# bobochow/adapt-image-models

Measured on AMD Instinct MI355X. Metric: clips/sec (8-frame 224^2 ViT-B/16 AIM fwd+bwd), higher is better.
Workload: dtype bf16; 1 GPU; BASELINE configs[1]: ViT-B/16 + AIM adapters, 8 frames 224^2, 64 clips/GPU, K400-shaped synthetic clips (400 random labels), fwd+bwd+AdamW; global_batch=64, frames=8, parallelism=dp1

## Files before the change

### adapt-image-models_amd/backbone.py

```python
import logging
import os
from collections import OrderedDict
from typing import Dict, List, Optional

import torch
from torch import nn

from . import ops
from .registry import BACKBONES

BF16, F32 = torch.bfloat16, torch.float32
_LOG = logging.getLogger("aim_amd")


def get_root_logger():
    return _LOG


class Adapter(nn.Module):

    def __init__(self, D_features: int, mlp_ratio: float = 0.25, skip_connect: bool = True):
        super().__init__()
        self.skip_connect = skip_connect
        hidden = int(D_features * mlp_ratio)
        self.D_fc1 = nn.Linear(D_features, hidden)
        self.D_fc2 = nn.Linear(hidden, D_features)


class LayerNorm(nn.LayerNorm):
    """Parameter container; the fp32 LayerNorm itself runs in ``aim_layernorm_fwd`` (vit_clip.py:71-77)."""


class QuickGELU(nn.Module):
    """Placeholder so ``mlp`` keeps the reference's three-entry Sequential (vit_clip.py:80-82,93-97)."""


class ResidualAttentionBlock(nn.Module):

    def __init__(self, d_model: int, n_head: int, scale: float = 1., num_frames: int = 8, drop_path: float = 0.):
        super().__init__()
        self.attn = nn.MultiheadAttention(d_model, n_head)
        self.ln_1 = LayerNorm(d_model)
        self.mlp = nn.Sequential(OrderedDict([
            ("c_fc", nn.Linear(d_model, d_model * 4)),
            ("gelu", QuickGELU()),
            ("c_proj", nn.Linear(d_model * 4, d_model))]))
        self.ln_2 = LayerNorm(d_model)
        self.n_head = n_head
        self.d_model = d_model
        self.MLP_Adapter = Adapter(d_model, skip_connect=False)
        self.S_Adapter = Adapter(d_model, skip_connect=False)
        self.scale = scale
        self.T_Adapter = Adapter(d_model, skip_connect=False)
        self.num_frames = num_frames
        self.drop_prob = float(drop_path)


class Transformer(nn.Module):
    def __init__(self, num_frames, width, layers, heads, scale=1., drop_path=0.1):
        super().__init__()
        self.width, self.layers = width, layers
        dpr = [x.item() for x in torch.linspace(0, drop_path, layers)]
        self.resblocks = nn.Sequential(*[
            ResidualAttentionBlock(width, heads, scale, num_frames, dpr[i]) for i in range(layers)])


_ADAPTERS = ("MLP_Adapter", "S_Adapter", "T_Adapter")
_ADAPTER_LEAVES = ("D_fc1.weight", "D_fc1.bias", "D_fc2.weight", "D_fc2.bias")


def _cast(w: torch.Tensor, transpose: bool = False) -> torch.Tensor:
    w2 = w.detach().reshape(w.shape[0], -1).contiguous().float()
    R, C = w2.shape
    out = torch.empty((C, R) if transpose else (R, C), dtype=BF16, device=w.device)
    ops.cast_bf16(w2, out, transpose)
    return out


class _Frozen:

    def __init__(self, blk: ResidualAttentionBlock):
        a = blk.attn
        self.Wqkv, self.WqkvT = _cast(a.in_proj_weight), _cast(a.in_proj_weight, True)
        self.Wo, self.WoT = _cast(a.out_proj.weight), _cast(a.out_proj.weight, True)
        D = blk.d_model
        r = blk.MLP_Adapter.D_fc1.weight.shape[0]
        dev = a.in_proj_weight.device
        self.D, self.r, self.H4 = D, r, 4 * D
        self.Wcat1 = torch.empty((4 * D + r, D), dtype=BF16, device=dev)
        self.Wcat2 = torch.empty((D, 4 * D + r), dtype=BF16, device=dev)
        self.WcatT2 = torch.empty((4 * D + r, D), dtype=BF16, device=dev)
        self.WcatT1 = torch.empty((D, 4 * D + r), dtype=BF16, device=dev)
        wfc, wpr = blk.mlp.c_fc.weight.detach().float().contiguous(), blk.mlp.c_proj.weight.detach().float().contiguous()
        ops.cast_bf16(wfc, self.Wcat1[:4 * D])
        ops.cast_bf16(wpr, self.Wcat2[:, :4 * D])
        ops.cast_bf16(wpr, self.WcatT2[:4 * D], transpose=True)
        ops.cast_bf16(wfc, self.WcatT1[:, :4 * D], transpose=True)
        self.bcat1 = torch.zeros(4 * D + r, dtype=F32, device=dev)
        self.bcat1[:4 * D] = blk.mlp.c_fc.bias.detach().float()
        self.small = {a: dict(W1=torch.empty((r, D), dtype=BF16, device=dev), W1T=torch.empty((D, r), dtype=BF16, device=dev),
                              W2=torch.empty((D, r), dtype=BF16, device=dev), W2T=torch.empty((r, D), dtype=BF16, device=dev))
                      for a in ("S_Adapter", "T_Adapter")}
        f = lambda p: p.detach().float().contiguous()
        self.bqkv, self.bo = f(a.in_proj_bias), f(a.out_proj.bias)
        self.bpr = f(blk.mlp.c_proj.bias)
        self.g1, self.b1 = f(blk.ln_1.weight), f(blk.ln_1.bias)
        self.g2, self.b2 = f(blk.ln_2.weight), f(blk.ln_2.bias)


    def cast_entries(self, name, w1, w2, b1=None):
        H4 = self.H4
        if name == "MLP_Adapter":
            ent = [(w1, self.Wcat1[H4:], False), (w2, self.Wcat2[:, H4:], False),
                   (w2, self.WcatT2[H4:], True), (w1, self.WcatT1[:, H4:], True)]
            if b1 is not None:
                ent.append((b1.reshape(1, -1), self.bcat1[H4:].reshape(1, -1), 2))
            return ent
        b = self.small[name]
        return [(w1, b["W1"], False), (w1, b["W1T"], True), (w2, b["W2"], False), (w2, b["W2T"], True)]

    def stage_mlp_adapter(self, w1, b1, w2, b2):
        for src, dst, tr in self.cast_entries("MLP_Adapter", w1.detach().float().contiguous(),
                                              w2.detach().float().contiguous()):
            ops.cast_bf16(src, dst, transpose=tr)
        self.stage_mlp_bias(b1, b2)

    def stage_mlp_bias(self, b1, b2, copy_b1: bool = True):
        if copy_b1:
            self.bcat1[self.H4:] = b1.detach().float()
        self.b2row = b2.detach().float().reshape(1, -1).contiguous()


class _Frozen8:

    def __init__(self, blk: ResidualAttentionBlock):
        a, ma = blk.attn, blk.MLP_Adapter
        q = ops.quantize_fp8_rows
        self.Wqkv, self.sqkv = q(a.in_proj_weight)
        self.Wo, self.so = q(a.out_proj.weight)
        self.Wcat1, self.s1 = q(torch.cat([blk.mlp.c_fc.weight.detach().float(), ma.D_fc1.weight.detach().float()], 0))
        self.Wcat2, self.s2 = q(torch.cat([blk.mlp.c_proj.weight.detach().float(), ma.D_fc2.weight.detach().float()], 1))


class _AdapterW:

    def __init__(self, w1, b1, w2, b2, bufs=None):
        if bufs is None:
            self.W1, self.W1T = _cast(w1), _cast(w1, True)
            self.W2, self.W2T = _cast(w2), _cast(w2, True)
        else:
            self.W1, self.W1T, self.W2, self.W2T = bufs["W1"], bufs["W1T"], bufs["W2"], bufs["W2T"]
        self.b1, self.b2 = b1.detach().float().contiguous(), b2.detach().float().contiguous()


def _empty(shape, dtype, dev):
    return torch.empty(shape, dtype=dtype, device=dev)


class _Arena:

    def __init__(self, dev, nbytes: int):
        self.dev, self.chunk = dev, int(nbytes)
        self.buf = torch.empty(self.chunk, dtype=torch.uint8, device=dev)
        self.off = 0
        self.main = torch.cuda.current_stream(dev) if dev.type == "cuda" else None

    def take(self, shape, dtype):
        n = 1
        for d in shape:
            n *= int(d)
        nbytes = (n * _ELEM[dtype] + 255) // 256 * 256
        if self.off + nbytes > self.buf.numel():
            with torch.cuda.stream(self.main):
                self.buf = torch.empty(max(self.chunk, nbytes), dtype=torch.uint8, device=self.dev)
            self.off = 0
        v = self.buf[self.off:self.off + nbytes].view(dtype)[:n].view(shape)
        self.off += nbytes
        return v


_ELEM = {BF16: 2, F32: 4}


_SIDE = {}
_DETACHED = {}

_JOIN_STATS = [] if os.environ.get("AIM_JOIN_STATS") else None


def join_stats():
    out = {}
    for tag, e0, e1 in _JOIN_STATS or []:
        out[tag] = out.get(tag, 0.0) + e0.elapsed_time(e1)
    if _JOIN_STATS is not None:
        _JOIN_STATS.clear()
    return out
_USE_SIDE = os.environ.get("AIM_SIDE_STREAM", "1") != "0"
_LAMBDA_ON_SIDE = os.environ.get("AIM_LAMBDA_SIDE", "1") != "0"
_LATE_JOIN = os.environ.get("AIM_LATE_JOIN", "1") != "0"
_FSUM_IN_LN = os.environ.get("AIM_FSUM_IN_LN", "1") != "0"
_CLS_EARLY = os.environ.get("AIM_CLS_EARLY", "1") != "0"
_LAMBDA_FUSED = os.environ.get("AIM_LAMBDA_FUSED", "1") != "0"
_DETACH_WGRAD = os.environ.get("AIM_DETACH_WGRAD", "1") != "0"
_DETACH_BIG = os.environ.get("AIM_DETACH_BIG", "1") != "0"
_EXPSUM_DETACHED = os.environ.get("AIM_EXPSUM_DETACHED", "0") != "0"
_DETACHED_PRIORITY = int(os.environ.get("AIM_DETACHED_PRIORITY", "0"))
_AUX_GRAD = os.environ.get("AIM_AUX_GRAD", "1") != "0"
_AUX_FRAG = os.environ.get("AIM_AUX_FRAG", "1") != "0" and os.environ.get("AIM_GEMM_TILE", "") != "128"
_DP_RESERVE = int(os.environ.get("AIM_DP_RESERVE_CUS", "0"))
_FP8_RES16 = os.environ.get("AIM_FP8_RES16", "1") != "0"
_EXPSUM_BORDER = os.environ.get("AIM_EXPSUM_BORDER", "1") != "0"
_QKV_RESERVE = int(os.environ.get("AIM_QKV_RESERVE", "32"))


class _Fork:

    def __init__(self, dev, tag: str = ""):
        self.enabled = _USE_SIDE
        self.dev = dev
        self.tag = tag
        self.started = False
        if self.enabled:
            key = (dev.type, dev.index)
            if key not in _SIDE:
                _SIDE[key] = torch.cuda.Stream(device=dev, priority=int(os.environ.get("AIM_SIDE_PRIORITY", "-1")))
            self.side_stream = _SIDE[key]
            self.main = torch.cuda.current_stream(dev)

    def sync_main_to_side(self):
        if self.enabled and self.started:
            ev = torch.cuda.Event()
            ev.record(self.side_stream)
            if _JOIN_STATS is not None:
                e0, e1 = torch.cuda.Event(enable_timing=True), torch.cuda.Event(enable_timing=True)
                e0.record(self.main)
                self.main.wait_event(ev)
                e1.record(self.main)
                _JOIN_STATS.append((self.tag + "-mid", e0, e1))
                return
            self.main.wait_event(ev)

    def sync_side_to_main(self):
        if self.enabled:
            ev = torch.cuda.Event()
            ev.record(self.main)
            self.side_stream.wait_event(ev)

    def side(self):
        fork = self

        class _Section:
            def __enter__(self_inner):
                if fork.enabled:
                    if not fork.started:
                        fork.started = True
                        fork.sync_side_to_main()
                    self_inner.ctx = torch.cuda.stream(fork.side_stream)
                    self_inner.ctx.__enter__()
                    if _JOIN_STATS is not None:
                        self_inner.t0 = torch.cuda.Event(enable_timing=True)
                        self_inner.t0.record(fork.side_stream)
                return fork

            def __exit__(self_inner, *exc):
                if fork.enabled:
                    if _JOIN_STATS is not None:
                        t1 = torch.cuda.Event(enable_timing=True)
                        t1.record(fork.side_stream)
                        _JOIN_STATS.append((fork.tag + "-span", self_inner.t0, t1))
                    self_inner.ctx.__exit__(*exc)
                return False

        return _Section()

    def __enter__(self):
        self._sec = self.side()
        return self._sec.__enter__()

    def __exit__(self, *exc):
        return self._sec.__exit__(*exc)

    def run_detached(self, calls: list, keep: list):
        if not calls:
            return
        if not (self.enabled and _DETACH_WGRAD):
            ctx = self.side() if self.enabled else None
            if ctx is not None:
                with ctx:
                    for f in calls:
                        f()
            else:
                for f in calls:
                    f()
            return
        key = (self.dev.type, self.dev.index)
        if key not in _DETACHED:
            _DETACHED[key] = torch.cuda.Stream(device=self.dev, priority=_DETACHED_PRIORITY)
        w = _DETACHED[key]
        ev = torch.cuda.Event()
        ev.record(self.side_stream)
        w.wait_event(ev)
        with torch.cuda.stream(w):
            for f in calls:
                f()
        keep.extend(calls)

    def run_beside(self, fn):
        if not self.enabled:
            fn()
            return None
        key = (self.dev.type, self.dev.index)
        if key not in _DETACHED:
            _DETACHED[key] = torch.cuda.Stream(device=self.dev, priority=_DETACHED_PRIORITY)
        w = _DETACHED[key]
        ev = torch.cuda.Event()
        ev.record(self.main)
        w.wait_event(ev)
        with torch.cuda.stream(w):
            fn()
        done = torch.cuda.Event()
        done.record(w)
        return done

    @staticmethod
    def streams(dev):
        key = (dev.type, dev.index)
        out = [torch.cuda.current_stream(dev)]
        for table in (_SIDE, _DETACHED):
            if key in table:
                out.append(table[key])
        return out

    @staticmethod
    def join_detached(dev):
        w = _DETACHED.get((dev.type, dev.index))
        if w is not None:
            ev = torch.cuda.Event()
            ev.record(w)
            main = torch.cuda.current_stream(dev)
            if _JOIN_STATS is not None:
                e0, e1 = torch.cuda.Event(enable_timing=True), torch.cuda.Event(enable_timing=True)
                e0.record(main)
                main.wait_event(ev)
                e1.record(main)
                _JOIN_STATS.append(("detached", e0, e1))
                return
            main.wait_event(ev)

    def join(self):
        if self.enabled and self.started:
            done = torch.cuda.Event()
            done.record(self.side_stream)
            if _JOIN_STATS is not None:
                e0, e1 = torch.cuda.Event(enable_timing=True), torch.cuda.Event(enable_timing=True)
                e0.record(self.main)
                self.main.wait_event(done)
                e1.record(self.main)
                _JOIN_STATS.append((self.tag, e0, e1))
                return
            self.main.wait_event(done)


def _adapter_fwd_small(x_bf, ad: _AdapterW, rows, r, D, ar: _Arena, out_f32: bool):
    pre, h = ar.take((rows, r), BF16), ar.take((rows, r), BF16)
    ops.gemm(x_bf, ad.W1, ops.EPI_ACT, h, bias=ad.b1, out2=pre, act=ops.ACT_GELU, aux_grad=_AUX_GRAD)
    out = ar.take((rows, D), F32 if out_f32 else BF16)
    ops.gemm(h, ad.W2, ops.EPI_F32 if out_f32 else ops.EPI_BF16, out, bias=ad.b2)
    return out, pre, h


def _block_forward(x, fz: _Frozen, adp: Dict[str, _AdapterW], B, T, N, H, dms1, dms2, save: bool, f8: Optional[_Frozen8] = None):
    assert f8 is None or not save
    dev = x.device
    M, D = x.shape
    BT = B * T
    r = fz.r
    fork = _Fork(dev, "fwd")
    ar = _Arena(dev, 48 * BT * D + 4 * B * H * T * T + 8 * BT * N + (1 << 16))

    def cls_chain(qkv_src, n_stride):
        ot = ar.take((BT, D), BF16)
        probs = ar.take((B, H, T, T), F32)
        ops.cls_attn_fwd(qkv_src, ot, probs, B, T, n_stride, H)
        ta = ar.take((BT, D), BF16)
        ops.gemm(ot, fz.Wo, ops.EPI_BF16, ta, bias=fz.bo)
        xt, t_pre, t_h = _adapter_fwd_small(ta, adp["T_Adapter"], BT, r, D, ar, out_f32=False)
        kv = ar.take((BT, 2 * D), BF16)
        ops.gemm(xt, fz.Wqkv[D:], ops.EPI_BF16, kv, bias=fz.bqkv[D:])
        crs = ar.take((BT, D), F32)
        ops.gemm(kv[:, D:], fz.Wo, ops.EPI_F32, crs, bias=fz.bo)
        return probs, ta, t_pre, t_h, kv, crs

    if _CLS_EARLY:
        with fork.side():
            xl_cls = ar.take((BT, D), BF16)
            if x.dtype == BF16:
                ops.layernorm_fwd_x16(x, fz.g1, fz.b1, BT, D, N * D, y_bf16=xl_cls)
            else:
                ops.layernorm_fwd(x, fz.g1, fz.b1, BT, D, N * D, y_bf16=xl_cls, mean=ar.take((BT,), F32),
                                  rstd=ar.take((BT,), F32))
            qkv_cls = ar.take((BT, 3 * D), BF16)
            ops.gemm(xl_cls, fz.Wqkv, ops.EPI_BF16, qkv_cls, bias=fz.bqkv)
            probs, ta, t_pre, t_h, kv, crs = cls_chain(qkv_cls, 1)
    qkv = _empty((M, 3 * D), BF16, dev)
    reserve = _QKV_RESERVE if (_CLS_EARLY and fork.enabled) else 0
    if f8 is not None:
        xl = _empty((M, D), ops.FP8, dev)
        mean1 = rstd1 = None
        if x.dtype == BF16:
            ops.layernorm_fwd_x16(x, fz.g1, fz.b1, M, D, D, y8=xl)
        else:
            ops.layernorm_fwd_fp8(x, fz.g1, fz.b1, M, D, D, xl)
        ops.gemm_fp8(xl, f8.Wqkv, f8.sqkv, ops.EPI_BF16, qkv, bias=fz.bqkv, reserve_cus=reserve)
    else:
        xl = _empty((M, D), BF16, dev)
        mean1, rstd1 = _empty((M,), F32, dev), _empty((M,), F32, dev)
        ops.layernorm_fwd(x, fz.g1, fz.b1, M, D, D, y_bf16=xl, mean=mean1, rstd=rstd1)
        ops.gemm(xl, fz.Wqkv, ops.EPI_BF16, qkv, bias=fz.bqkv, reserve_cus=reserve)
    del xl
    if not _CLS_EARLY:
        with fork.side():
            probs, ta, t_pre, t_h, kv, crs = cls_chain(qkv, N)
    fused = _LAMBDA_FUSED and _CLS_EARLY and N < 256 and ops.expsum_tiles(N, N) == 8
    ss, part_ready = None, None
    if fused:
        fork.sync_main_to_side()
        nt = 16
        part = _empty((BT, nt, 2), F32, dev)
        ops.gemm(qkv, qkv[:, D:], ops.EPI_EXPSUM, part, M=N, N=N, K=D, batch=BT, stride_a=N * 3 * D,
                 stride_w=N * 3 * D, scale=0.125, xrow=kv)
    else:
        border = (_EXPSUM_BORDER and N == 257 and D in (512, 1024) and _LAMBDA_ON_SIDE and _CLS_EARLY
                  and ops.expsum_tiles(N - 1, N - 1) == 8)
        nt = 10 if border else ops.expsum_tiles(N, N)
        part = _empty((BT, nt, 2), F32, dev)
        if _LAMBDA_ON_SIDE and _CLS_EARLY:
            fork.sync_side_to_main()
            with fork.side():
                ss = ar.take((BT, N), F32)
                if border:
                    ops.qk_border(qkv, kv, ss, part, 8, BT, N, D, 0.125)
                else:
                    ops.qk_cross(qkv, kv, ss, BT, N, D, 0.125)

        def expsum():
            if border:
                ops.gemm(qkv, qkv[:, D:], ops.EPI_EXPSUM, part, M=N - 1, N=N - 1, K=D, batch=BT, stride_a=N * 3 * D,
                         stride_w=N * 3 * D, scale=0.125, slot_stride=2 * nt)
            else:
                ops.gemm(qkv, qkv[:, D:], ops.EPI_EXPSUM, part, M=N, N=N, K=D, batch=BT, stride_a=N * 3 * D,
                         stride_w=N * 3 * D, scale=0.125)

        part_ready = fork.run_beside(expsum) if _EXPSUM_DETACHED else expsum()

    def lamda_chain():
        lam, oml = ar.take((BT,), F32), ar.take((BT,), F32)
        if fused:
            ops.lambda_partials(part, lam, oml, BT)
        else:
            ops.lambda_(qkv, kv, part, nt, lam, oml, BT, N, D, 0.125, ss=ss)
        sin = ar.take((BT, D), BF16)
        ops.scale_rows(crs, lam, y=sin)
        return (lam, oml, sin) + _adapter_fwd_small(sin, adp["S_Adapter"], BT, r, D, ar, out_f32=True)

    if _LAMBDA_ON_SIDE:
        if part_ready is not None:
            fork.side_stream.wait_event(part_ready)
        else:
            fork.sync_side_to_main()
        with fork.side():
            lam, oml, sin, sv, s_pre, s_h = lamda_chain()
    if f8 is not None:
        ao, lse = _empty((M, D), ops.FP8, dev), None
        ops.attn_fwd_fp8(qkv, ao, BT, N, H)
    else:
        ao = _empty((M, D), BF16, dev)
        lse = _empty((BT, H, N), F32, dev)
        ops.attn_fwd(qkv, ao, lse, BT, N, H)
    fork.join()
    if not _LAMBDA_ON_SIDE:
        if part_ready is not None:
            torch.cuda.current_stream(dev).wait_event(part_ready)
        lam, oml, sin, sv, s_pre, s_h = lamda_chain()
    H4 = 4 * D
    if f8 is not None:
        r16 = x.dtype == BF16
        epi_res, rdt = (ops.EPI_RES16, BF16) if r16 else (ops.EPI_F32, F32)
        x1 = _empty((M, D), rdt, dev)
        ops.gemm_fp8(ao, f8.Wo, f8.so, epi_res, x1, bias=fz.bo, resid=x, af=oml, vec=sv, bt=dms1, ntok=N)
        xn = _empty((M, D), ops.FP8, dev)
        if r16:
            ops.layernorm_fwd_x16(x1, fz.g2, fz.b2, M, D, D, y8=xn)
        else:
            ops.layernorm_fwd_fp8(x1, fz.g2, fz.b2, M, D, D, xn)
        hcat = _empty((M, H4 + r), ops.FP8, dev)
        ops.gemm_fp8(xn, f8.Wcat1, f8.s1, ops.EPI_ACT8, hcat, bias=fz.bcat1, act=ops.ACT_QGELU, n_split=H4,
                     act2=ops.ACT_GELU, at=dms2, ntok=N)
        x2 = _empty((M, D), rdt, dev)
        ops.gemm_fp8(hcat, f8.Wcat2, f8.s2, epi_res, x2, bias=fz.bpr, resid=x1, vec=fz.b2row, ldv=0, bt=dms2, ntok=N)
        return x2, None
    x1 = _empty((M, D), F32, dev)
    ops.gemm(ao, fz.Wo, ops.EPI_F32, x1, bias=fz.bo, resid=x, af=oml, vec=sv, bt=dms1, ntok=N)
    x2, xn, mean2, rstd2, hcat_pre, a_s = _mlp_adapter_forward(x1, fz, dms2, N, save)
    ctx = None
    if save:
        ctx = dict(x=x, mean1=mean1, rstd1=rstd1, qkv=qkv, probs=probs, ta=ta, t_pre=t_pre, t_h=t_h, lam=lam,
                   oml=oml, ao=ao, lse=lse, sin=sin, s_pre=s_pre, s_h=s_h, x1=x1, mean2=mean2, rstd2=rstd2, xn=xn,
                   hcat_pre=hcat_pre, a_s=a_s, dms1=dms1, dms2=dms2)
    return x2, ctx


def _mlp_adapter_forward(x1, fz: _Frozen, dms2, N, save: bool):
    dev = x1.device
    M, D = x1.shape
    r, H4 = fz.r, 4 * D
    xn = _empty((M, D), BF16, dev)
    mean2, rstd2 = _empty((M,), F32, dev), _empty((M,), F32, dev)
    ops.layernorm_fwd(x1, fz.g2, fz.b2, M, D, D, y_bf16=xn, mean=mean2, rstd=rstd2)
    frag = _AUX_FRAG and M >= 1024
    if frag:
        hcat_pre = ops.frag_buffer(M, H4 + r, dev) if save else None
    else:
        hcat_pre = _empty((M, H4 + r), BF16, dev) if (save or M < 1024) else None
    hcat = _empty((M, H4 + r), BF16, dev)
    ops.gemm(xn, fz.Wcat1, ops.EPI_ACT, hcat, bias=fz.bcat1, out2=hcat_pre, act=ops.ACT_QGELU, n_split=H4,
             act2=ops.ACT_GELU, at=dms2, ntok=N, aux_grad=_AUX_GRAD, aux_frag=frag and hcat_pre is not None)
    x2 = _empty((M, D), F32, dev)
    ops.gemm(hcat, fz.Wcat2, ops.EPI_F32, x2, bias=fz.bpr, resid=x1, vec=fz.b2row, ldv=0, bt=dms2, ntok=N)
    a_s = hcat[:, H4:] if save else None
    return x2, xn, mean2, rstd2, hcat_pre, a_s


def _mlp_adapter_backward(dyb, x_in, mean2, rstd2, xn, hcat_pre, a_s, dms2, fz: _Frozen, gm, N, fsum=None):
    dev = dyb.device
    M, D = dyb.shape
    r, H4 = fz.r, 4 * D
    big_later: list = []
    if _DETACH_BIG:
        big_later.append(lambda: ops.wgrad(dyb, a_s, gm["D_fc2.weight"], gm["D_fc2.bias"], at=dms2, ntok=N))
    else:
        ops.wgrad(dyb, a_s, gm["D_fc2.weight"], gm["D_fc2.bias"], at=dms2, ntok=N)
    dcat = _empty((M, H4 + r), BF16, dev)
    ops.gemm(dyb, fz.WcatT2, ops.EPI_DACT, dcat, aux=hcat_pre, act=ops.ACT_QGELU, n_split=H4, act2=ops.ACT_GELU,
             at=dms2, ntok=N, aux_grad=_AUX_GRAD, aux_frag=_AUX_FRAG and dyb.shape[0] >= 1024, reserve_cus=_DP_RESERVE)
    if _DETACH_BIG:
        big_later.append(lambda: ops.wgrad(dcat[:, H4:], xn, gm["D_fc1.weight"], gm["D_fc1.bias"]))
    else:
        ops.wgrad(dcat[:, H4:], xn, gm["D_fc1.weight"], gm["D_fc1.bias"])
    dxn = _empty((M, D), BF16, dev)
    ops.gemm(dcat, fz.WcatT1, ops.EPI_BF16, dxn, reserve_cus=_DP_RESERVE)
    dxb = _empty((M, D), BF16, dev)
    if fsum is not None:
        ops.layernorm_bwd_fsum(dxn, x_in, fz.g2, mean2, rstd2, dyb, dxb, fsum[0], fsum[1], M // N, N, D)
    else:
        ops.layernorm_bwd(dxn, x_in, fz.g2, mean2, rstd2, M, D, lddy=D, ldx=D, lddx=D, dres=dyb, dx_bf16=dxb)
    return dxb, big_later


def _adapter_bwd_small(dout_bf, ad: _AdapterW, a_in, pre, h, grads, rows, r, D, ar: _Arena, need_dx_bf16: bool, later: list):
    later.append(lambda: ops.wgrad(dout_bf, h, grads["D_fc2.weight"], grads["D_fc2.bias"]))
    dpre = ar.take((rows, r), BF16)
    ops.gemm(dout_bf, ad.W2T, ops.EPI_DACT, dpre, aux=pre, act=ops.ACT_GELU, aux_grad=_AUX_GRAD)
    later.append(lambda: ops.wgrad(dpre, a_in, grads["D_fc1.weight"], grads["D_fc1.bias"]))
    din = ar.take((rows, D), BF16 if need_dx_bf16 else F32)
    ops.gemm(dpre, ad.W1T, ops.EPI_BF16 if need_dx_bf16 else ops.EPI_F32, din)
    return din


def _block_backward(dyb, c, fz: _Frozen, adp: Dict[str, _AdapterW], grads, B, T, N, H, keep: Optional[list] = None):
    dev = dyb.device
    M, D = dyb.shape
    BT = B * T
    r, H4 = fz.r, 4 * D
    fpart = _empty((BT, ops.LN_FSUM_GROUPS, D), F32, dev) if _FSUM_IN_LN else None
    dx1b, big_later = _mlp_adapter_backward(dyb, c["x1"], c["mean2"], c["rstd2"], c["xn"], c["hcat_pre"], c["a_s"], c["dms2"],
                                            fz, grads["MLP_Adapter"], N, fsum=(c["dms1"], fpart) if _FSUM_IN_LN else None)
    later: list = big_later
    ar = _Arena(dev, 48 * BT * D + (1 << 16))
    with _Fork(dev, "bwd") as fork:
        dsv = ar.take((BT, D), F32)
        if _FSUM_IN_LN:
            ops.frame_sum(fpart, None, dsv, BT, ops.LN_FSUM_GROUPS, D)
        else:
            ops.frame_sum(dx1b, c["dms1"], dsv, BT, N, D)
        dsv_b = ar.take((BT, D), BF16)
        ops.cast_bf16(dsv, dsv_b)
        dsin = _adapter_bwd_small(dsv_b, adp["S_Adapter"], c["sin"], c["s_pre"], c["s_h"], grads["S_Adapter"], BT, r,
                                  D, ar, need_dx_bf16=False, later=later)
        dcrs = ar.take((BT, D), BF16)
        ops.scale_rows(dsin, c["lam"], y=dcrs)
        dvx = ar.take((BT, D), BF16)
        ops.gemm(dcrs, fz.WoT, ops.EPI_BF16, dvx)
        dxt = ar.take((BT, D), BF16)
        ops.gemm(dvx, fz.WqkvT[:, 2 * D:], ops.EPI_BF16, dxt)
        dta = _adapter_bwd_small(dxt, adp["T_Adapter"], c["ta"], c["t_pre"], c["t_h"], grads["T_Adapter"], BT, r, D,
                                 ar, need_dx_bf16=True, later=later)
        dot = ar.take((BT, D), BF16)
        ops.gemm(dta, fz.WoT, ops.EPI_BF16, dot)
        if _LATE_JOIN:
            dqkv_cls = ar.take((BT, 3 * D), BF16)
            ops.cls_attn_bwd(c["qkv"], c["probs"], dot, dqkv_cls, B, T, N, H, compact=True)
            dxl_cls = ar.take((BT, D), F32)
            ops.gemm(dqkv_cls, fz.WqkvT, ops.EPI_F32, dxl_cls)
    if keep is None:
        keep = []
        fork.run_detached(later, keep)
        _Fork.join_detached(dev)
    else:
        fork.run_detached(later, keep)
    dao = _empty((M, D), BF16, dev)
    ops.gemm(dx1b, fz.WoT, ops.EPI_BF16, dao, af=c["oml"], ntok=N, reserve_cus=_DP_RESERVE)
    dqkv = _empty((M, 3 * D), BF16, dev)
    delta = _empty((BT, H, N), F32, dev)
    ops.attn_bwd(c["qkv"], c["ao"], dao, c["lse"], delta, dqkv, BT, N, H)
    del dao
    if not _LATE_JOIN:
        fork.join()
        ops.cls_attn_bwd(c["qkv"], c["probs"], dot, dqkv, B, T, N, H)
    dxl = _empty((M, D), BF16, dev)
    ops.gemm(dqkv, fz.WqkvT, ops.EPI_BF16, dxl, reserve_cus=_DP_RESERVE)
    del dqkv
    if _LATE_JOIN:
        fork.join()
        ops.add_rows(dxl, N * D, dxl_cls)
    dxb = _empty((M, D), BF16, dev)
    ops.layernorm_bwd(dxl, c["x"], fz.g1, c["mean1"], c["rstd1"], M, D, lddy=D, ldx=D, lddx=D, dres=dx1b, dx_bf16=dxb)
    return dxb


class _BackboneFn(torch.autograd.Function):

    @staticmethod
    def forward(ctx, model: "ViT_CLIP", grad_enabled: bool, imgs: torch.Tensor, *params: torch.Tensor):
        L, H = model.layers, model.heads
        B, C, T, Hh, Ww = imgs.shape
        D, p = model.width, model.patch_size
        G = Hh // p
        N = G * G + 1
        BT, M = B * T, B * T * N
        dev = imgs.device
        temporal, lnp_w, lnp_b = params[0], params[1], params[2]
        need_grad = grad_enabled and any(ctx.needs_input_grad)
        frozen = model._frozen_operands()
        staged_bias = model._stage_adapters(frozen, params)
        adp = []
        for i in range(L):
            d = {}
            for j, a in enumerate(_ADAPTERS):
                k = 3 + (i * 3 + j) * 4
                if a == "MLP_Adapter":
                    frozen["blocks"][i].stage_mlp_bias(params[k + 1], params[k + 3], copy_b1=not staged_bias)
                else:
                    d[a] = _AdapterW(params[k], params[k + 1], params[k + 2], params[k + 3],
                                     bufs=frozen["blocks"][i].small[a])
            adp.append(d)
        Kp = frozen["conv"].shape[1]
        A = _empty((BT * G * G, Kp), BF16, dev)
        blend, model._blend_now = model._blend_now, None
        if blend is not None:
            ops.patchify_blend(imgs, A, B, T, Hh, Ww, p, Kp, *model._norm_now, blend=blend)
        else:
            ops.patchify(imgs, A, B, T, Hh, Ww, p, Kp, *model._norm_now)
        tok = _empty((BT * G * G, D), BF16, dev)
        ops.gemm(A, frozen["conv"], ops.EPI_BF16, tok)
        del A
        x = _empty((M, D), F32, dev)
        mean0, rstd0 = _empty((M,), F32, dev), _empty((M,), F32, dev)
        tmp = temporal.detach().reshape(T, D).float().contiguous()
        ops.embed_ln(tok, frozen["cls"], frozen["pos"], tmp, frozen["gpre"], frozen["bpre"], x, mean0, rstd0, B, T, N, D)
        ctxs: List[Optional[dict]] = []
        training = model.training
        f8 = None
        if model.inference_precision == 'fp8' and not need_grad:
            if M >= 1024 and model.variant == 'vit_clip':
                f8 = model._fp8_operands()
            elif not getattr(model, "_fp8_warned", False):
                model._fp8_warned = True
                _LOG.warning("fp8 inference was requested but this forward runs bf16: %s",
                             "the stock-AIM variant has no fp8 path" if model.variant != 'vit_clip'
                             else "fewer than 1024 token rows (M = %d)" % M)
        masks = model._drop_masks(N, training, dev)
        aim = model.variant == 'aim'
        if aim:
            from .aim_variant import aim_block_forward
        ckpt = bool(model.checkpoint) and need_grad

        def run_block(i, x_in, save):
            dms1, dms2 = masks[i, 0], masks[i, 1]
            if aim:
                scale = float(model.transformer.resblocks[i].scale)
                return aim_block_forward(x_in, frozen["blocks"][i], adp[i], B, T, N, H, dms1 * (1.0 / scale), dms2, save)
            return _block_forward(x_in, frozen["blocks"][i], adp[i], B, T, N, H, dms1, dms2, save,
                                  f8=None if f8 is None else f8[i])

        if f8 is not None and _FP8_RES16:
            x16 = _empty((M, D), BF16, dev)
            ops.cast_bf16(x, x16)
            x = x16
        for i in range(L):
            x_in = x
            x, c = run_block(i, x_in, need_grad and not ckpt)
            ctxs.append(dict(recompute=run_block, x_in=x_in) if ckpt else c)
        gw, gb = lnp_w.detach().float().contiguous(), lnp_b.detach().float().contiguous()
        y = _empty((BT, D), F32, dev)
        meanp, rstdp = _empty((BT,), F32, dev), _empty((BT,), F32, dev)
        if x.dtype == BF16:
            ops.layernorm_fwd_x16(x, gw, gb, BT, D, N * D, y_f32=y)
        else:
            ops.layernorm_fwd(x, gw, gb, BT, D, N * D, y_f32=y, mean=meanp, rstd=rstdp)
        if need_grad:
            ctx.model, ctx.dims = model, (B, T, N, H, D, L)
            ctx.saved = dict(ctxs=ctxs, adp=adp, tok=tok, mean0=mean0, rstd0=rstd0, tmp=tmp, xL=x, gw=gw, meanp=meanp,
                             rstdp=rstdp, params=params)
        return y.reshape(B, T, D).permute(0, 2, 1)

    @staticmethod
    def backward(ctx, dout):
        model = ctx.model
        B, T, N, H, D, L = ctx.dims
        s = ctx.saved
        BT, M = B * T, B * T * N
        dev = dout.device
        frozen = model._frozen_operands()
        params = s["params"]
        grads_out: List[Optional[torch.Tensor]] = [None] * len(params)
        in_place = [False] * len(params)

        def buf(k):
            p_ = params[k]
            if (model.grad_in_place and p_.requires_grad and p_.grad is not None and p_.grad.dtype == F32
                    and p_.grad.is_contiguous() and p_.grad.device == dev):
                in_place[k] = True
                return p_.grad
            return torch.zeros_like(p_, dtype=F32)

        layer_grads = []
        for i in range(L):
            lg = {}
            for j, a in enumerate(_ADAPTERS):
                k = 3 + (i * 3 + j) * 4
                lg[a] = {}
                for e, leaf in enumerate(_ADAPTER_LEAVES):
                    g = buf(k + e)
                    lg[a][leaf] = g
                    grads_out[k + e] = g
            layer_grads.append(lg)
        dgw, dgb = buf(1), buf(2)
        dy = dout.permute(0, 2, 1).reshape(BT, D).contiguous().float()
        dxb = torch.zeros((M, D), dtype=BF16, device=dev)
        ops.layernorm_bwd(dy, s["xL"], s["gw"], s["meanp"], s["rstdp"], BT, D, lddy=D, ldx=N * D, lddx=N * D,
                          dx_bf16=dxb, dgamma=dgw, dbeta=dgb)
        keep: list = []
        hook = model.grad_ready_hook
        blk_bwd = _block_backward
        if model.variant == 'aim':
            from .aim_variant import aim_block_backward as blk_bwd
        for i in reversed(range(L)):
            c = s["ctxs"][i]
            if "recompute" in c:
                c = c["recompute"](i, c["x_in"], True)[1]
            recomputed = "recompute" in s["ctxs"][i]
            dxb = blk_bwd(dxb, c, frozen["blocks"][i], s["adp"][i], layer_grads[i], B, T, N, H, keep)
            s["ctxs"][i] = c = None
            if recomputed:
                _Fork.join_detached(dev)
                keep.clear()
            if hook is not None:
                k0 = 3 + i * 12
                hook(i, all(in_place[k0:k0 + 12]), _Fork.streams(dev))
        dtmp = buf(0)
        ops.embed_bwd(dxb, s["tok"], frozen["cls"], frozen["pos"], s["tmp"], frozen["gpre"], s["mean0"], s["rstd0"],
                      dtmp.view(T, D), B, T, N, D)
        grads_out[0] = dtmp.view(1, T, D)
        grads_out[1], grads_out[2] = dgw, dgb
        _Fork.join_detached(dev)
        keep.clear()
        for k, p_ in enumerate(params):
            if not p_.requires_grad or in_place[k]:
                grads_out[k] = None
            elif grads_out[k] is not None and grads_out[k].dtype != p_.dtype:
                grads_out[k] = grads_out[k].to(p_.dtype)
        ctx.saved = None
        return (None, None, None) + tuple(grads_out)


@BACKBONES.register_module()
class ViT_CLIP(nn.Module):

    def __init__(self, input_resolution: int, num_frames: int, patch_size: int, width: int, layers: int, heads: int,
                 drop_path_rate, adapter_scale=0.5, pretrained=None, shift=False, checkpoint=False):
        super().__init__()
        if shift:
            raise NotImplementedError("ViT_CLIP(shift=True) is dead code in the reference and is not supported")
        if width % heads != 0 or width // heads != 64:
            raise ValueError("the HIP attention kernels are built for head_dim 64 (ViT-B/16, ViT-L/14)")
        self.input_resolution = input_resolution
        self.pretrained = pretrained
        self.patch_size = patch_size
        self.width, self.layers, self.heads = width, layers, heads
        self.conv1 = nn.Conv2d(in_channels=3, out_channels=width, kernel_size=patch_size, stride=patch_size, bias=False)
        scale = width ** -0.5
        self.class_embedding = nn.Parameter(scale * torch.randn(width))
        self.positional_embedding = nn.Parameter(scale * torch.randn((input_resolution // patch_size) ** 2 + 1, width))
        self.ln_pre = LayerNorm(width)
        self.num_frames = num_frames
        self.temporal_embedding = nn.Parameter(torch.zeros(1, num_frames, width))
        self.shift = shift
        self.checkpoint = checkpoint
        self.transformer = Transformer(num_frames, width, layers, heads, scale=adapter_scale, drop_path=drop_path_rate)
        self.ln_post = LayerNorm(width)
        self._frozen_cache = None
        self._norm_mean = self._norm_std = None
        self._norm_now = (None, None)
        self._blend_next = None
        self._blend_now = None
        self.grad_in_place = False
        self.grad_ready_hook = None
        self._fp8_cache = None
        self.weights_epoch = 0
        self.variant = 'vit_clip'
        self.inference_precision = 'fp8' if os.environ.get("AIM_INFER_FP8", "0") == "1" else 'bf16'
        self._cast_table = None
        self.precision = 'bf16'

    def set_precision(self, precision: str):
        if precision not in ('bf16', 'fp32'):
            raise ValueError("precision must be 'bf16' or 'fp32'")
        self.precision = precision
        return self

    def init_weights(self, pretrained=None):
        def _init_weights(m):
            if isinstance(m, nn.Linear):
                nn.init.trunc_normal_(m.weight, std=.02)
                if m.bias is not None:
                    nn.init.constant_(m.bias, 0)
            elif isinstance(m, nn.LayerNorm):
                nn.init.constant_(m.bias, 0)
                nn.init.constant_(m.weight, 1.0)

        if pretrained:
            self.pretrained = pretrained
        if isinstance(self.pretrained, str):
            self.apply(_init_weights)
            try:
                import clip
            except ImportError as e:
                raise RuntimeError(
                    "pretrained=%r needs the OpenAI `clip` package and its downloaded weights "
                    "(reference vit_clip.py:369-372); load a CLIP visual state_dict with "
                    "load_state_dict(strict=False) instead" % (self.pretrained,)) from e
            name = "ViT-B/16" if self.layers == 12 else "ViT-L/14"
            clip_model, _ = clip.load(name, device="cpu")
            sd = clip_model.visual.state_dict()
            del clip_model
            del sd['proj']
            msg = self.load_state_dict(sd, strict=False)
            _LOG.info('Missing keys: %s', msg.missing_keys)
            _LOG.info('Unexpected keys: %s', msg.unexpected_keys)
        elif self.pretrained is None:
            self.apply(_init_weights)
        else:
            raise TypeError('pretrained must be a str or None')
        for n, m in self.transformer.named_modules():
            if n.split(".")[-1] in _ADAPTERS:
                nn.init.constant_(m.D_fc2.weight, 0)
                nn.init.constant_(m.D_fc2.bias, 0)
        for name, param in self.named_parameters():
            if ('temporal_embedding' not in name and 'ln_post' not in name and 'Adapter' not in name
                    and 'cls_head' not in name):
                param.requires_grad = False
        n_train = sum(p.numel() for p in self.parameters() if p.requires_grad)
        n_total = sum(p.numel() for p in self.parameters())
        _LOG.info('Number of total parameters: %6.2f, tunable parameters: %6.2f', n_total / 1e6, n_train / 1e6)
        self._frozen_cache = None

    @torch.jit.ignore
    def no_weight_decay(self):
        return {'absolute_pos_embed', 'temporal_embedding'}

    @torch.jit.ignore
    def no_weight_decay_keywords(self):
        return {'relative_position_bias_table', 'temporal_position_bias_table'}

    def _param_slots(self, root, tag):
        cache = self.__dict__.setdefault("_slot_cache", {})
        if tag not in cache:
            cache[tag] = [(m, n) for m in root.modules() for n in m._parameters if m._parameters[n] is not None]
        return [m._parameters[n] for m, n in cache[tag]]

    def _frozen_params(self):
        skip = set(id(p) for p in self._trainable_list())
        return [p for p in self._param_slots(self, "all") if id(p) not in skip]

    def _frozen_operands(self):
        key = tuple((p.data_ptr(), p._version) for p in self._frozen_params())
        if self._frozen_cache is not None and self._frozen_cache[0] == key:
            return self._frozen_cache[1]
        D, p = self.width, self.patch_size
        K = 3 * p * p
        Kp = (K + 63) // 64 * 64
        dev = self.conv1.weight.device
        wc = torch.zeros((D, Kp), dtype=F32, device=dev)
        wc[:, :K] = self.conv1.weight.detach().reshape(D, K).float()
        conv = torch.empty((D, Kp), dtype=BF16, device=dev)
        ops.cast_bf16(wc, conv)
        f = lambda t: t.detach().float().contiguous()
        out = dict(conv=conv, cls=f(self.class_embedding), pos=f(self.positional_embedding),
                   gpre=f(self.ln_pre.weight), bpre=f(self.ln_pre.bias),
                   blocks=[_Frozen(b) for b in self.transformer.resblocks])
        self._frozen_cache = (key, out)
        return out

    def set_inference_precision(self, precision: str):
        if precision not in ('bf16', 'fp8'):
            raise ValueError("inference precision must be 'bf16' or 'fp8'")
        self.inference_precision = precision
        return self

    def _fp8_operands(self):
        key = tuple((p.data_ptr(), p._version) for p in self._param_slots(self.transformer, "blocks")) + (self.weights_epoch,)
        if self._fp8_cache is None or self._fp8_cache[0] != key:
            self._fp8_cache = (key, [_Frozen8(b) for b in self.transformer.resblocks])
        return self._fp8_cache[1]

    def _stage_adapters(self, frozen, params):
        srcs = []
        for i in range(self.layers):
            for j, a in enumerate(_ADAPTERS):
                k = 3 + (i * 3 + j) * 4
                srcs += [params[k], params[k + 2]]
                if a == "MLP_Adapter":
                    srcs.append(params[k + 1])
        ok = all(p.dtype == F32 and p.is_contiguous() for p in srcs)
        key = tuple(p.data_ptr() for p in srcs) + (id(frozen),)
        if ok and (self._cast_table is None or self._cast_table[0] != key):
            entries = []
            for i in range(self.layers):
                for j, a in enumerate(_ADAPTERS):
                    k = 3 + (i * 3 + j) * 4
                    entries += frozen["blocks"][i].cast_entries(a, params[k].detach(), params[k + 2].detach(),
                                                                params[k + 1].detach() if a == "MLP_Adapter" else None)
            self._cast_table = (key, ops.CastTable(entries, srcs[0].device))
        if ok:
            self._cast_table[1].run()
            return True
        for i in range(self.layers):
            for j, a in enumerate(_ADAPTERS):
                k = 3 + (i * 3 + j) * 4
                for src, dst, tr in frozen["blocks"][i].cast_entries(a, params[k].detach().float().contiguous(),
                                                                     params[k + 2].detach().float().contiguous()):
                    ops.cast_bf16(src, dst, transpose=tr)
        return False

    def _trainable_list(self):
        ps = [self.temporal_embedding, self.ln_post.weight, self.ln_post.bias]
        for blk in self.transformer.resblocks:
            for a in _ADAPTERS:
                m = getattr(blk, a)
                ps += [m.D_fc1.weight, m.D_fc1.bias, m.D_fc2.weight, m.D_fc2.bias]
        return ps

    @staticmethod
    def _drop_mask(N, drop_prob, scale, training, dev):
        if drop_prob > 0. and training:
            keep = 1.0 - drop_prob
            m = torch.empty(N, dtype=F32, device=dev).bernoulli_(keep)
            return m.div_(keep).mul_(scale) if keep > 0 else m.mul_(0.)
        return torch.full((N,), float(scale), dtype=F32, device=dev)

    def _drop_masks(self, N, training, dev):
        blocks = self.transformer.resblocks
        L = len(blocks)
        key = (str(dev), tuple(float(b.drop_prob) for b in blocks), tuple(float(b.scale) for b in blocks))
        cached = getattr(self, "_drop_consts", None)
        if cached is None or cached[0] != key:
            rates = torch.tensor(key[1], dtype=F32)
            scale = torch.tensor(key[2], dtype=F32)
            keep = 1.0 - rates
            fac = torch.where(keep > 0, scale / keep.clamp_min(1e-12), torch.zeros_like(keep))
            cached = (key, float(rates.max()), scale.to(dev).view(L, 1, 1), keep.to(dev).view(L, 1, 1), fac.to(dev).view(L, 1, 1))
            self._drop_consts = cached
        _, max_rate, scale_d, keep_d, fac_d = cached
        if not training or max_rate <= 0.:
            return scale_d.expand(L, 2, N).contiguous()
        u = torch.rand((L, 2, N), dtype=F32, device=dev)
        return (u < keep_d).to(F32) * fac_d

    def forward(self, x: torch.Tensor):
        blend, self._blend_next = self._blend_next, None
        if not x.is_cuda:
            raise RuntimeError("aim_amd.ViT_CLIP runs on MI355X only (HIP kernels); there is no CPU fallback")
        B, C, T, H, W = x.shape
        if T != self.num_frames:
            raise ValueError(f"expected {self.num_frames} frames, got {T}")
        if C != 3 or H != self.input_resolution or W != self.input_resolution:
            raise ValueError(f"expected input [B,3,{T},{self.input_resolution},{self.input_resolution}], got {tuple(x.shape)}")
        if x.dtype == torch.float16:
            x = x.float()
        x = x.contiguous()
        self._norm_now = (self._norm_mean, self._norm_std) if x.dtype == torch.uint8 else (None, None)
        self._norm_mean = self._norm_std = None
        if x.dtype == torch.uint8 and self._norm_now[0] is None:
            raise TypeError("uint8 clips need a GPUNormalize module hook on the backbone (module_hooks.py:35-87)")
        if blend is not None and (x.dtype not in (torch.float32, torch.uint8) or blend.partner.numel() != B):
            raise TypeError(f"a fused blending needs float32 or uint8 clips and one partner per clip, got {x.dtype} and "
                            f"{blend.partner.numel()} partners for {B} clips")
        self._blend_now = blend
        if self.precision == 'fp32':
            from .fp32_path import _BackboneFn32, forward_f32
            if torch.is_grad_enabled() and any(p.requires_grad for p in self._trainable_list()):
                return _BackboneFn32.apply(self, x, *self._trainable_list()).unsqueeze(-1).unsqueeze(-1)
            with torch.no_grad():
                return forward_f32(self, x).unsqueeze(-1).unsqueeze(-1)
        y = _BackboneFn.apply(self, torch.is_grad_enabled(), x, *self._trainable_list())
        return y.unsqueeze(-1).unsqueeze(-1)
```

### adapt-image-models_amd/csrc/wgrad.hip

```cpp
#include "aim_common.h"
#include <stdlib.h>
#include "aim_kernels_internal.h"

namespace {

constexpr int MSTEP = 32;
constexpr int NST = 4;
constexpr int IMG = MSTEP * 128;
constexpr int OPER_BYTES = 4 * IMG;
constexpr int STAGE_BYTES = 2 * OPER_BYTES;
constexpr int TILE = 256;

__global__ __launch_bounds__(512) void wgrad_kernel(const bf16_t* __restrict__ G, int ldg, const bf16_t* __restrict__ A,
                                                    int lda, float* __restrict__ dW, int lddw, float* __restrict__ partial,
                                                    int M, int Nw, int Kw, int chunk, float* __restrict__ db,
                                                    float* __restrict__ bias_partial, const float* __restrict__ at, int ntok) {
    extern __shared__ __attribute__((aligned(16))) char smem_raw[];
    AIM_LDS char* smem = (AIM_LDS char*)smem_raw;
    AIM_LDS float* sAt = (AIM_LDS float*)(smem + NST * STAGE_BYTES);
    const int tiles_k = (Kw + TILE - 1) / TILE;
    const int tiles = ((Nw + TILE - 1) / TILE) * tiles_k;
    const int cidx = blockIdx.x / tiles, tix = blockIdx.x - cidx * tiles;
    const int tn = tix / tiles_k, tk = tix - tn * tiles_k;
    const int n0 = tn * TILE, k0 = tk * TILE;
    const int mbeg = cidx * chunk;
    const int mend = min(M, mbeg + chunk);
    if (mbeg >= mend) return;

    const int tid = threadIdx.x, lane = tid & 63;
    const int wave = __builtin_amdgcn_readfirstlane(tid >> 6);
    const int wn = wave >> 2, wk = wave & 3;
    const int frow = lane & 15, fq = lane >> 4;

    const bf16_t* Gb = G + (long long)mbeg * ldg + n0;
    const bf16_t* Ab = A + (long long)mbeg * lda + k0;
    const int rows = mend - mbeg;
    aim_rsrc_words rG = make_rsrc_words(Gb, ((long long)(rows - 1) * ldg + min(TILE, Nw - n0)) * 2);
    aim_rsrc_words rA = make_rsrc_words(Ab, ((long long)(rows - 1) * lda + min(TILE, Kw - k0)) * 2);

    const int srow = lane >> 3, schunk = (lane & 7) ^ srow;
    unsigned vg0[2], va0[2];
    AIM_LDS char* pdst[2];
#pragma unroll
    for (int j = 0; j < 2; ++j) {
        const int piece = wave * 2 + j;
        const int img = piece >> 2, rg = piece & 3;
        const int r = rg * 8 + srow;
        const int col = img * 64 + schunk * 8;
        vg0[j] = n0 + col < Nw ? (unsigned)((r * ldg + col) * 2) : AIM_OOB;
        va0[j] = k0 + col < Kw ? (unsigned)((r * lda + col) * 2) : AIM_OOB;
        pdst[j] = smem + img * IMG + rg * 1024;
    }
    const unsigned gstep = (unsigned)(MSTEP * ldg * 2), astep = (unsigned)(MSTEP * lda * 2);
    auto stage = [&](int buf, int ms) {
#pragma unroll
        for (int j = 0; j < 2; ++j) {
            stage_piece_asm(rG, pdst[j] + buf * STAGE_BYTES, vg0[j] + (unsigned)ms * gstep);
            stage_piece_asm(rA, pdst[j] + buf * STAGE_BYTES + OPER_BYTES, va0[j] + (unsigned)ms * astep);
        }
    };

    f32x4 acc[8][4];
#pragma unroll
    for (int i = 0; i < 8; ++i)
#pragma unroll
        for (int j = 0; j < 4; ++j) acc[i][j] = f32x4{0.f, 0.f, 0.f, 0.f};

    auto frag = [&](const AIM_LDS char* oper, int c0) -> bf16x8 {
        const AIM_LDS char* img = oper + (c0 >> 6) * IMG;
        const int ch = ((c0 & 63) >> 3) + ((frow & 3) >> 1), half8 = (frow & 1) * 8;
        const int r0 = fq * 4 + (frow >> 2);
        const bf16x4 a = lds_read_tr4(img + swz_off(r0, ch) + half8);
        const bf16x4 b = lds_read_tr4(img + swz_off(r0 + 16, ch) + half8);
        bf16x8 f;
#pragma unroll
        for (int e = 0; e < 4; ++e) {
            f[e] = a[e];
            f[4 + e] = b[e];
        }
        return f;
    };

    const int nsteps = (rows + MSTEP - 1) / MSTEP;
    const bool do_bias = db != nullptr && tk == 0;
    float bs[8] = {0.f, 0.f, 0.f, 0.f, 0.f, 0.f, 0.f, 0.f};
    const int bcg = tid & 31, brow = tid >> 5;
    int btok0 = 0, btok1 = 0;
    if (do_bias && at) {
        for (int i = tid; i < ntok; i += 512) sAt[i] = at[i];
        asm volatile("s_waitcnt lgkmcnt(0)" ::: "memory");
        btok0 = (mbeg + brow) % ntok;
        btok1 = (mbeg + brow + 16) % ntok;
    }
    const int bstep = MSTEP % (ntok > 0 ? ntok : 1);
    stage(0, 0); stage(1, 1); stage(2, 2);
    for (int ms = 0; ms < nsteps; ++ms) {
        asm volatile("s_waitcnt vmcnt(8)" ::: "memory");
        __builtin_amdgcn_s_barrier();
        stage((ms + 3) % NST, ms + 3);
        const AIM_LDS char* sG = smem + (ms % NST) * STAGE_BYTES;
        const AIM_LDS char* sA = sG + OPER_BYTES;
        if (do_bias) {
            const AIM_LDS char* img = sG + (bcg >> 3) * IMG;
            const bf16x8 v0 = lds_read8(img + swz_off(brow, bcg & 7));
            const bf16x8 v1 = lds_read8(img + swz_off(brow + 16, bcg & 7));
            float f0 = 1.0f, f1 = 1.0f;
            if (at) {
                f0 = sAt[btok0];
                f1 = sAt[btok1];
                btok0 += bstep; if (btok0 >= ntok) btok0 -= ntok;
                btok1 += bstep; if (btok1 >= ntok) btok1 -= ntok;
            }
#pragma unroll
            for (int e = 0; e < 8; ++e) bs[e] += f0 * (float)v0[e] + f1 * (float)v1[e];
        }
        bf16x8 gf[8], af[4];
#pragma unroll
        for (int j = 0; j < 4; ++j) af[j] = frag(sA, wk * 64 + j * 16);
#pragma unroll
        for (int i = 0; i < 8; ++i) gf[i] = frag(sG, wn * 128 + i * 16);
#pragma unroll
        for (int i = 0; i < 8; ++i)
#pragma unroll
            for (int j = 0; j < 4; ++j)
                acc[i][j] = __builtin_amdgcn_mfma_f32_16x16x32_bf16(af[j], gf[i], acc[i][j], 0, 0, 0);
    }
    asm volatile("s_waitcnt vmcnt(0)" ::: "memory");
    if (do_bias) {
        __syncthreads();
        AIM_LDS float* red = (AIM_LDS float*)smem;
#pragma unroll
        for (int e = 0; e < 8; ++e) red[brow * 256 + bcg * 8 + e] = bs[e];
        __syncthreads();
        if (tid < 256 && n0 + tid < Nw) {
            float v = 0.f;
#pragma unroll
            for (int r = 0; r < 16; ++r) v += red[r * 256 + tid];
            if (bias_partial) bias_partial[(long long)cidx * Nw + n0 + tid] = v;
            else db[n0 + tid] += v;
        }
    }
    float* slab = partial ? partial + (long long)cidx * Nw * Kw : nullptr;
#pragma unroll
    for (int i = 0; i < 8; ++i)
#pragma unroll
        for (int j = 0; j < 4; ++j) {
            const int n = n0 + wn * 128 + i * 16 + frow;
            const int k = k0 + wk * 64 + j * 16 + fq * 4;
            if (n >= Nw || k >= Kw) continue;
            if (slab) *(f32x4*)(slab + (long long)n * Kw + k) = acc[i][j];
            else
#pragma unroll
                for (int e = 0; e < 4; ++e) atomicAdd(dW + (long long)n * lddw + k + e, acc[i][j][e]);
        }
}

__global__ __launch_bounds__(256) void wgrad_finish_kernel(const float* __restrict__ partial, float* __restrict__ dW,
                                                           int lddw, int nchunks, int Nw, int Kw,
                                                           const float* __restrict__ bias_partial, float* __restrict__ db) {
    const long long total = (long long)Nw * Kw;
    const long long idx = ((long long)blockIdx.x * 256 + threadIdx.x) * 4;
    if (idx < total) {
        f32x4 acc = f32x4{0.f, 0.f, 0.f, 0.f};
        int c = 0;
        for (; c + 8 <= nchunks; c += 8) {
            f32x4 v[8];
#pragma unroll
            for (int j = 0; j < 8; ++j) v[j] = *(const f32x4*)(partial + (long long)(c + j) * total + idx);
#pragma unroll
            for (int j = 0; j < 8; ++j) acc += v[j];
        }
        for (; c < nchunks; ++c) acc += *(const f32x4*)(partial + (long long)c * total + idx);
        const int n = (int)(idx / Kw), k = (int)(idx - (long long)n * Kw);
        f32x4* o = (f32x4*)(dW + (long long)n * lddw + k);
        *o = *o + acc;
    }
    if (bias_partial) {
        const int n = blockIdx.x * 4 + (threadIdx.x >> 6), lane = threadIdx.x & 63;
        if (n < Nw) {
            float a = 0.f;
            for (int c = lane; c < nchunks; c += 64) a += bias_partial[(long long)c * Nw + n];
            a = wave_sum(a);
            if (lane == 0) db[n] += a;
        }
    }
}

__global__ __launch_bounds__(256) void wgrad_finish1_kernel(const float* __restrict__ partial, float* __restrict__ dW,
                                                            int lddw, int nchunks, int Nw, int Kw) {
    const long long idx = (long long)blockIdx.x * 256 + threadIdx.x;
    const long long total = (long long)Nw * Kw;
    if (idx >= total) return;
    float acc = 0.f;
    for (int c = 0; c < nchunks; ++c) acc += partial[(long long)c * total + idx];
    const int n = (int)(idx / Kw), k = (int)(idx - (long long)n * Kw);
    dW[(long long)n * lddw + k] += acc;
}

}

static int wgrad_chunks(int M, int tiles, int* chunk_out) {
    static const int target = [] { const char* e = getenv("AIM_WGRAD_WGS"); const int v = e ? atoi(e) : 256; return v > 0 ? v : 256; }();
    int nchunks = (target + tiles - 1) / tiles;
    const int maxchunks = (M + MSTEP - 1) / MSTEP;
    if (nchunks > maxchunks) nchunks = maxchunks;
    int chunk = (M + nchunks - 1) / nchunks;
    chunk = ((chunk + MSTEP - 1) / MSTEP) * MSTEP;
    if (chunk_out) *chunk_out = chunk;
    return (M + chunk - 1) / chunk;
}

extern "C" int64_t aim_wgrad_workspace_bytes(int M, int Nw, int Kw) {
    const int tiles = ((Nw + TILE - 1) / TILE) * ((Kw + TILE - 1) / TILE);
    const int nchunks = wgrad_chunks(M, tiles, nullptr);
    return nchunks > 1 ? (int64_t)nchunks * Nw * (Kw + 1) * 4 : 0;
}

extern "C" int aim_wgrad_bias_bf16(const aim_bf16* G, int ldg, const aim_bf16* A, int lda, float* dW, int lddw, float* db,
                                   const float* at, int ntok, int M, int Nw, int Kw, float* workspace, int64_t workspace_bytes,
                                   void* stream) {
    AIM_CHECK_ARG(M > 0 && Nw > 0 && Kw > 0 && (Nw % 8) == 0 && (Kw % 8) == 0, "wgrad: Nw/Kw must be positive multiples of 8 (Nw=%d Kw=%d)", Nw, Kw);
    AIM_CHECK_ARG((ldg % 8) == 0 && (lda % 8) == 0 && (lddw % 4) == 0, "wgrad: ldg/lda must be multiples of 8, lddw of 4");
    AIM_CHECK_ARG(G && A && dW, "wgrad: null pointer");
    AIM_CHECK_ARG(!at || (db && ntok > 0 && ntok <= 4096), "wgrad: row factors need db and 0 < ntok <= 4096");
    const int tiles = ((Nw + TILE - 1) / TILE) * ((Kw + TILE - 1) / TILE);
    int chunk = 0;
    const int nchunks = wgrad_chunks(M, tiles, &chunk);
    const int lds_bytes = NST * STAGE_BYTES + (at ? ((ntok * 4 + 15) & ~15) : 0);
    static bool attr_set = false;
    if (!attr_set) {
        (void)hipFuncSetAttribute((const void*)wgrad_kernel, hipFuncAttributeMaxDynamicSharedMemorySize, 160 * 1024);
        attr_set = true;
    }
    AIM_CHECK_ARG((long long)chunk * (ldg > lda ? ldg : lda) * 2 < 0x7fffffffLL, "wgrad: chunk too large");
    float* slab = (workspace && nchunks > 1 && workspace_bytes >= (int64_t)nchunks * Nw * (Kw + 1) * 4) ? workspace : nullptr;
    static const bool fuse_bias = [] { const char* e = getenv("AIM_WGRAD_FUSE_BIAS"); return !e || atoi(e) != 0; }();
    static const bool finish_v = [] { const char* e = getenv("AIM_WGRAD_FINISH_V"); return !e || atoi(e) != 0; }();
    float* bias_slab = (slab && db && fuse_bias) ? slab + (long long)nchunks * Nw * Kw : nullptr;
    if (db && nchunks > 1 && !bias_slab) {
        const int rc = aim_colsum_bf16(G, ldg, nullptr, at, ntok, db, M, Nw, nullptr, 0, stream);
        if (rc) return rc;
        db = nullptr;
    }
    hipLaunchKernelGGL(wgrad_kernel, dim3(tiles * nchunks), dim3(512), lds_bytes, (hipStream_t)stream,
                       (const bf16_t*)G, ldg, (const bf16_t*)A, lda, dW, lddw, slab, M, Nw, Kw, chunk, db, bias_slab, at, ntok);
    AIM_CHECK_LAUNCH("aim_wgrad_bf16");
    if (slab) {
        const long long total = (long long)Nw * Kw;
        unsigned fgrid = (unsigned)((total / 4 + 255) / 256);
        if (bias_slab && (unsigned)((Nw + 3) / 4) > fgrid) fgrid = (unsigned)((Nw + 3) / 4);
        if (finish_v || bias_slab)
            hipLaunchKernelGGL(wgrad_finish_kernel, dim3(fgrid), dim3(256), 0, (hipStream_t)stream,
                               slab, dW, lddw, nchunks, Nw, Kw, bias_slab, db);
        else
            hipLaunchKernelGGL(wgrad_finish1_kernel, dim3((unsigned)((total + 255) / 256)), dim3(256), 0, (hipStream_t)stream,
                               slab, dW, lddw, nchunks, Nw, Kw);
        AIM_CHECK_LAUNCH("aim_wgrad_bf16(finish)");
    }
    return 0;
}

extern "C" int aim_wgrad_bf16(const aim_bf16* G, int ldg, const aim_bf16* A, int lda, float* dW, int lddw, float* db,
                              int M, int Nw, int Kw, float* workspace, int64_t workspace_bytes, void* stream) {
    return aim_wgrad_bias_bf16(G, ldg, A, lda, dW, lddw, db, nullptr, 0, M, Nw, Kw, workspace, workspace_bytes, stream);
}
```

### adapt-image-models_amd/lib.py

```python
import ctypes
import os
from ctypes import POINTER, Structure, c_char_p, c_float, c_int, c_int32, c_int64, c_void_p

_HERE = os.path.dirname(os.path.abspath(__file__))
_LIB = None


class LibraryNotBuilt(RuntimeError):
    pass


def library_path() -> str:
    return os.environ.get("AIM_HIP_LIB") or os.path.join(_HERE, "libaim_hip.so")


class GemmArgs(Structure):
    _fields_ = [
        ("A", c_void_p), ("W", c_void_p), ("lda", c_int32), ("ldw", c_int32),
        ("strideA", c_int64), ("strideW", c_int64),
        ("M", c_int32), ("N", c_int32), ("K", c_int32),
        ("bias", c_void_p), ("resid", c_void_p), ("ldr", c_int32),
        ("af", c_void_p), ("at", c_void_p), ("vec", c_void_p), ("bt", c_void_p),
        ("ldv", c_int32), ("ntok", c_int32),
        ("aux", c_void_p), ("ldaux", c_int32),
        ("out", c_void_p), ("ldo", c_int32), ("out2", c_void_p), ("ldo2", c_int32),
        ("scale", c_float), ("act", c_int32), ("rs_bias_only", c_int32), ("n_split", c_int32), ("act2", c_int32),
        ("xrow", c_void_p), ("ldx", c_int32),
        ("reserve_cus", c_int32), ("probe", c_void_p), ("probe_cap", c_int32),
        ("wscale", c_void_p), ("aux_grad", c_int32), ("aux_frag", c_int32), ("row0", c_int32),
    ]


P = c_void_p
I = c_int
L = c_int64
F = c_float

SIGNATURES = {
    "aim_version": [],
    "aim_last_error": [],
    "aim_gemm_bf16": [POINTER(GemmArgs), I, I, P],
    "aim_gemm_fp8": [POINTER(GemmArgs), I, P],
    "aim_gemm_expsum_tiles": [I, I],
    "aim_wgrad_bf16": [P, I, P, I, P, I, P, I, I, I, P, L, P],
    "aim_wgrad_workspace_bytes": [I, I, I],
    "aim_wgrad_bias_bf16": [P, I, P, I, P, I, P, P, I, I, I, I, P, L, P],
    "aim_layernorm_fwd": [P, L, P, P, P, P, L, P, P, I, I, F, P],
    "aim_layernorm_fwd_fp8": [P, L, P, P, P, L, I, I, F, P],
    "aim_layernorm_fwd_x16": [P, L, P, P, P, P, P, L, I, I, F, P],
    "aim_layernorm_bwd": [P, I, L, P, L, P, P, P, P, I, P, P, L, P, P, I, I, P],
    "aim_layernorm_bwd_fsum": [P, L, P, L, P, P, P, P, P, L, P, P, I, I, I, I, P],
    "aim_attn_fwd": [P, P, P, I, I, I, P],
    "aim_attn_fwd_fp8": [P, P, P, I, I, I, P],
    "aim_attn_bwd": [P, P, P, P, P, P, I, I, I, P],
    "aim_cls_attn_fwd": [P, P, P, I, I, I, I, P],
    "aim_cls_attn_bwd": [P, P, P, P, I, I, I, I, I, P],
    "aim_tattn_fwd": [P, P, P, I, I, I, I, P],
    "aim_tattn_bwd": [P, P, P, P, I, I, I, I, P],
    "aim_add_bf16": [P, L, P, L, P, L, I, I, P],
    "aim_acc_bf16": [P, P, L, I, I, P],
    "aim_lambda_partials": [P, P, P, I, P],
    "aim_qk_cross": [P, P, I, P, I, I, I, F, P],
    "aim_lambda": [P, P, I, P, P, I, P, P, I, I, I, F, P],
    "aim_qk_border": [P, P, I, P, P, I, I, I, I, I, F, P],
    "aim_patchify": [P, I, P, P, P, I, I, I, I, I, I, P],
    "aim_patchify_blend": [P, I, P, P, P, I, I, I, I, I, I, P, I, F, F, I, I, I, I, P],
    "aim_embed_ln": [P, P, P, P, P, P, P, P, P, I, I, I, I, F, P],
    "aim_embed_bwd": [P, I, P, P, P, P, P, P, P, P, I, I, I, I, P, L, P],
    "aim_embed_bwd_workspace_bytes": [I, I, I, I],
    "aim_frame_sum": [P, I, P, P, I, I, I, P],
    "aim_colsum_bf16": [P, I, P, P, I, P, I, I, P, L, P],
    "aim_cast_bf16": [P, P, I, I, I, I, P],
    "aim_scale_rows": [P, P, P, P, I, I, P],
    "aim_add_rows_bf16": [P, L, P, I, I, P],
    "aim_adamw_flat": [P, P, P, P, L, F, F, F, F, F, I, F, P],
    "aim_head_fwd": [P, P, P, P, P, P, I, I, I, I, P],
    "aim_head_bwd": [P, P, P, P, P, P, P, I, I, I, I, P],
    "aim_ce_topk": [P, P, P, P, P, I, I, I, P],
    "aim_ce_soft": [P, P, P, P, P, P, I, I, P],
    "aim_cast_multi": [P, I, P],
    "aim_gemm_f32": [POINTER(GemmArgs), I, I, P],
    "aim_attn_fwd_f32": [P, P, I, I, I, P],
    "aim_cls_attn_fwd_f32": [P, L, P, I, I, I, P],
    "aim_lambda_f32": [P, I, P, P, I, P, P, I, I, I, F, P],
    "aim_patchify_f32": [P, I, P, P, P, I, I, I, I, I, I, P],
    "aim_patchify_blend_f32": [P, I, P, P, P, I, I, I, I, I, I, P, I, F, F, I, I, I, I, P],
    "aim_embed_ln_f32": [P, P, P, P, P, P, P, P, P, P, I, I, I, I, F, P],
    "aim_attn_bwd_f32_workspace_bytes": [I, I, I],
    "aim_attn_bwd_f32": [P, P, P, I, I, I, P, L, P],
    "aim_cls_attn_bwd_f32": [P, L, P, P, I, I, I, P],
    "aim_tattn_fwd_f32": [P, P, I, I, I, I, P],
    "aim_tattn_bwd_f32": [P, P, P, I, I, I, I, P],
    "aim_wgrad_f32_workspace_bytes": [I, I, I],
    "aim_wgrad_f32": [P, I, P, I, P, I, I, I, P, P, I, P, L, P],
    "aim_embed_nopre_fwd": [P, P, P, P, P, I, I, I, I, P],
    "aim_embed_nopre_bwd_workspace_bytes": [I, I, I, I],
    "aim_embed_nopre_bwd": [P, I, P, P, P, P, P, I, I, I, I, P, L, P],
    "aim_layernorm_gb_bwd_workspace_bytes": [I, I],
    "aim_layernorm_gb_bwd": [P, I, L, P, L, P, P, P, P, I, I, P, L, P],
}

ABI_VERSION = 8


def load_library():
    global _LIB
    if _LIB is not None:
        return _LIB
    path = library_path()
    if not os.path.exists(path):
        raise LibraryNotBuilt(
            f"{path} not found: build it with `python -c 'import __graft_entry__ as g; g.build()'` "
            f"(or `make -C adapt-image-models_amd/csrc`). There is no CPU fallback.")
    lib = ctypes.CDLL(path)
    for name, argtypes in SIGNATURES.items():
        fn = getattr(lib, name)
        fn.argtypes = argtypes
        fn.restype = c_char_p if name == "aim_last_error" else (c_int64 if name.endswith("_bytes") else c_int)
    if lib.aim_version() != ABI_VERSION:
        raise LibraryNotBuilt(f"{path}: ABI version {lib.aim_version()} != {ABI_VERSION}; rebuild")
    _LIB = lib
    return lib


def check(rc: int, what: str = ""):
    if rc != 0:
        msg = load_library().aim_last_error()
        raise RuntimeError(f"libaim_hip {what} failed (rc={rc}): {msg.decode() if msg else '?'}")
```

### adapt-image-models_amd/ops.py

```python
from ctypes import byref
from typing import Optional

import torch

from .lib import GemmArgs, check, load_library

EPI_BF16, EPI_ACT, EPI_DACT, EPI_F32, EPI_EXPSUM, EPI_ACT8, EPI_RES16 = 0, 1, 2, 3, 4, 5, 6
FP8 = torch.float8_e4m3fn
ACT_QGELU, ACT_GELU = 0, 1

BF16 = torch.bfloat16
F32 = torch.float32


_RAW_STREAM = getattr(torch._C, "_cuda_getCurrentRawStream", None)
_RAW_DEVICE = getattr(torch._C, "_cuda_getDevice", None)


def _stream() -> int:
    if _RAW_STREAM is not None:
        return _RAW_STREAM(_RAW_DEVICE())
    return torch.cuda.current_stream().cuda_stream


class KernelTimer:

    def __init__(self, min_flops: float = 1e10):
        self.min_flops = min_flops
        self.enabled = False
        self.records = []

    def start(self):
        self.records, self.enabled = [], True

    def stop(self):
        self.enabled = False

    def summary(self):
        out = {}
        for epi, fl, e0, e1 in self.records:
            d = out.setdefault(epi, dict(launches=0, flops=0.0, ms=0.0))
            d["launches"] += 1
            d["flops"] += fl
            d["ms"] += e0.elapsed_time(e1)
        return out


GEMM_TIMER = KernelTimer()


def _p(t: Optional[torch.Tensor]) -> Optional[int]:
    return None if t is None else t.data_ptr()


def _chk(t: Optional[torch.Tensor], dtype, name: str):
    if t is None:
        return
    if not t.is_cuda:
        raise RuntimeError(f"{name}: expected a GPU tensor (the HIP path has no CPU fallback)")
    if t.dtype != dtype:
        raise TypeError(f"{name}: expected {dtype}, got {t.dtype}")
    if t.dim() >= 1 and t.stride(-1) != 1:
        raise ValueError(f"{name}: innermost dimension must be contiguous")


def frag_elems(M: int, N: int) -> int:
    return ((M + 255) // 256) * ((N + 255) // 256) * 65536


def frag_buffer(M: int, N: int, device) -> torch.Tensor:
    return torch.empty((frag_elems(M, N),), dtype=BF16, device=device)


def gemm(a: torch.Tensor, w: torch.Tensor, epi: int, out: torch.Tensor, *, bias=None, resid=None,
         af=None, at=None, vec=None, bt=None, ntok: int = 0, aux=None, out2=None, act: int = 0,
         scale: float = 1.0, rs_bias_only: bool = False, batch: int = 1, stride_a: int = 0,
         stride_w: int = 0, M: Optional[int] = None, N: Optional[int] = None, K: Optional[int] = None,
         lda: Optional[int] = None, ldw: Optional[int] = None, ldv: Optional[int] = None, n_split: int = 0,
         act2: int = 0, xrow=None, reserve_cus: int = 0, probe=None, aux_grad: bool = False, aux_frag: bool = False,
         slot_stride: int = 0):
    lib = load_library()
    _chk(a, BF16, "a"); _chk(w, BF16, "w")
    for n_, t_ in (("bias", bias), ("resid", resid), ("af", af), ("at", at), ("vec", vec), ("bt", bt)):
        _chk(t_, F32, n_)
    _chk(aux, BF16, "aux"); _chk(out2, BF16, "out2")
    g = GemmArgs()
    g.A, g.W = a.data_ptr(), w.data_ptr()
    g.M = a.shape[0] if M is None else M
    g.K = a.shape[1] if K is None else K
    g.N = w.shape[0] if N is None else N
    g.lda = a.stride(0) if lda is None else lda
    g.ldw = w.stride(0) if ldw is None else ldw
    g.strideA, g.strideW = stride_a, stride_w
    g.bias, g.resid = _p(bias), _p(resid)
    g.ldr = resid.stride(0) if resid is not None else 0
    g.af, g.at, g.vec, g.bt = _p(af), _p(at), _p(vec), _p(bt)
    g.ldv = (vec.stride(0) if ldv is None else ldv) if vec is not None else 0
    g.ntok = ntok
    g.aux = _p(aux)
    g.ldaux = aux.stride(0) if aux is not None else 0
    g.out = out.data_ptr()
    g.ldo = (out.stride(0) if out.dim() >= 2 else 0) if epi != EPI_EXPSUM else int(slot_stride)
    g.out2 = _p(out2)
    g.ldo2 = out2.stride(0) if out2 is not None else 0
    g.scale, g.act, g.rs_bias_only = scale, act, int(rs_bias_only)
    g.n_split, g.act2 = n_split, act2
    _chk(xrow, BF16, "xrow")
    g.xrow = _p(xrow)
    g.ldx = xrow.stride(0) if xrow is not None else 0
    g.reserve_cus = int(reserve_cus)
    g.aux_grad = int(bool(aux_grad))
    g.aux_frag = int(bool(aux_frag))
    if aux_frag:
        t_ = out2 if epi == EPI_ACT else aux
        if epi not in (EPI_ACT, EPI_DACT) or batch != 1 or g.M < 1024 or t_ is None or not t_.is_contiguous() \
                or t_.numel() < frag_elems(g.M, g.N):
            raise ValueError("aux_frag: ACT / DACT on the large-tile kernel (M >= 1024, batch 1) with a frag_buffer(M, N)")
        g.ldo2 = g.ldaux = 0
    if probe is not None:
        g.probe, g.probe_cap = probe.data_ptr(), probe.shape[0]
    if epi in (EPI_BF16, EPI_ACT, EPI_DACT):
        _chk(out, BF16, "out")
    else:
        _chk(out, F32, "out")
    timed = GEMM_TIMER.enabled and 2.0 * g.M * g.N * g.K * batch >= GEMM_TIMER.min_flops
    if timed:
        e0, e1 = torch.cuda.Event(enable_timing=True), torch.cuda.Event(enable_timing=True)
        e0.record()
    check(lib.aim_gemm_bf16(byref(g), epi, batch, _stream()), "aim_gemm_bf16")
    if timed:
        e1.record()
        GEMM_TIMER.records.append((epi, 2.0 * g.M * g.N * g.K * batch, e0, e1))
    return out


def gemm_fp8(a8: torch.Tensor, w8: torch.Tensor, wscale: torch.Tensor, epi: int, out: torch.Tensor, *, bias=None,
             resid=None, af=None, at=None, vec=None, bt=None, ntok: int = 0, act: int = 0, n_split: int = 0, act2: int = 0,
             ldv: Optional[int] = None, reserve_cus: int = 0, probe=None):
    lib = load_library()
    for n_, t_ in (("a8", a8), ("w8", w8)):
        if not t_.is_cuda or t_.element_size() != 1 or t_.stride(-1) != 1:
            raise TypeError(f"{n_}: expected a GPU fp8 (1-byte) tensor with a contiguous last dimension")
    for n_, t_ in (("wscale", wscale), ("bias", bias), ("af", af), ("at", at), ("vec", vec), ("bt", bt)):
        _chk(t_, F32, n_)
    _chk(resid, BF16 if epi == EPI_RES16 else F32, "resid")
    g = GemmArgs()
    g.A, g.W = a8.data_ptr(), w8.data_ptr()
    g.M, g.K, g.N = a8.shape[0], a8.shape[1], w8.shape[0]
    g.lda, g.ldw = a8.stride(0), w8.stride(0)
    g.bias, g.resid, g.wscale = _p(bias), _p(resid), wscale.data_ptr()
    g.ldr = resid.stride(0) if resid is not None else 0
    g.af, g.at, g.vec, g.bt = _p(af), _p(at), _p(vec), _p(bt)
    g.ldv = (vec.stride(0) if ldv is None else ldv) if vec is not None else 0
    g.ntok = ntok
    g.out, g.ldo = out.data_ptr(), out.stride(0)
    g.act, g.n_split, g.act2, g.scale = act, n_split, act2, 1.0
    g.reserve_cus = int(reserve_cus)
    if probe is not None:
        g.probe, g.probe_cap = probe.data_ptr(), probe.shape[0]
    if epi in (EPI_BF16, EPI_RES16):
        _chk(out, BF16, "out")
    elif epi == EPI_F32:
        _chk(out, F32, "out")
    elif out.element_size() != 1:
        raise TypeError("out: EPI_ACT8 writes fp8 bytes")
    timed = GEMM_TIMER.enabled and 2.0 * g.M * g.N * g.K >= GEMM_TIMER.min_flops
    if timed:
        e0, e1 = torch.cuda.Event(enable_timing=True), torch.cuda.Event(enable_timing=True)
        e0.record()
    check(lib.aim_gemm_fp8(byref(g), epi, _stream()), "aim_gemm_fp8")
    if timed:
        e1.record()
        GEMM_TIMER.records.append((100 + epi, 2.0 * g.M * g.N * g.K, e0, e1))
    return out


def quantize_fp8_rows(w: torch.Tensor):
    wf = w.detach().float()
    amax = wf.abs().amax(dim=1).clamp_min(1e-12)
    scale = amax / 448.0
    q = (wf / scale[:, None]).clamp_(-448.0, 448.0)
    w8 = q.cpu().to(FP8).to(w.device)
    return w8.contiguous(), scale.contiguous()


def layernorm_fwd_fp8(x, gamma, beta, rows, D, ldx, y8, ldy=None, eps: float = 1e-5):
    _chk(x, F32, "x"); _chk(gamma, F32, "gamma"); _chk(beta, F32, "beta")
    if y8.element_size() != 1 or not y8.is_cuda:
        raise TypeError("y8: expected a GPU fp8 (1-byte) tensor")
    check(load_library().aim_layernorm_fwd_fp8(x.data_ptr(), ldx, gamma.data_ptr(), beta.data_ptr(), y8.data_ptr(),
                                               D if ldy is None else ldy, rows, D, eps, _stream()), "aim_layernorm_fwd_fp8")


def layernorm_fwd_x16(x, gamma, beta, rows, D, ldx, *, y_bf16=None, y_f32=None, y8=None, ldy=None, eps: float = 1e-5):
    _chk(x, BF16, "x"); _chk(gamma, F32, "gamma"); _chk(beta, F32, "beta"); _chk(y_bf16, BF16, "y_bf16"); _chk(y_f32, F32, "y_f32")
    if y8 is not None and (y8.element_size() != 1 or not y8.is_cuda):
        raise TypeError("y8: expected a GPU fp8 (1-byte) tensor")
    check(load_library().aim_layernorm_fwd_x16(x.data_ptr(), ldx, gamma.data_ptr(), beta.data_ptr(), _p(y_bf16), _p(y_f32), _p(y8),
                                               D if ldy is None else ldy, rows, D, eps, _stream()), "aim_layernorm_fwd_x16")


def attn_fwd_fp8(qkv, out8, BT, N, H, lse=None):
    _chk(qkv, BF16, "qkv"); _chk(lse, F32, "lse")
    if out8.element_size() != 1 or not out8.is_cuda:
        raise TypeError("out8: expected a GPU fp8 (1-byte) tensor")
    check(load_library().aim_attn_fwd_fp8(qkv.data_ptr(), out8.data_ptr(), _p(lse), BT, N, H, _stream()), "aim_attn_fwd_fp8")


def expsum_tiles(M: int, N: int) -> int:
    return load_library().aim_gemm_expsum_tiles(M, N)


def wgrad(g: torch.Tensor, a: torch.Tensor, dw: torch.Tensor, db: Optional[torch.Tensor] = None, at=None, ntok: int = 0):
    _chk(g, BF16, "g"); _chk(a, BF16, "a"); _chk(dw, F32, "dw"); _chk(db, F32, "db"); _chk(at, F32, "at")
    assert g.shape[0] == a.shape[0] and dw.shape == (g.shape[1], a.shape[1])
    lib = load_library()
    nbytes = lib.aim_wgrad_workspace_bytes(g.shape[0], g.shape[1], a.shape[1])
    ws = torch.empty(nbytes // 4, dtype=F32, device=g.device) if nbytes else None
    check(lib.aim_wgrad_bias_bf16(g.data_ptr(), g.stride(0), a.data_ptr(), a.stride(0), dw.data_ptr(), dw.stride(0), _p(db),
                                  _p(at), ntok, g.shape[0], g.shape[1], a.shape[1], _p(ws), nbytes, _stream()), "aim_wgrad_bias_bf16")


def layernorm_fwd(x, gamma, beta, rows, D, ldx, *, y_bf16=None, y_f32=None, ldy=None, mean=None, rstd=None,
                  eps: float = 1e-5):
    _chk(x, F32, "x"); _chk(gamma, F32, "gamma"); _chk(beta, F32, "beta")
    _chk(y_bf16, BF16, "y_bf16"); _chk(y_f32, F32, "y_f32"); _chk(mean, F32, "mean"); _chk(rstd, F32, "rstd")
    check(load_library().aim_layernorm_fwd(x.data_ptr(), ldx, gamma.data_ptr(), beta.data_ptr(), _p(y_bf16),
                                           _p(y_f32), D if ldy is None else ldy, _p(mean), _p(rstd), rows, D,
                                           eps, _stream()), "aim_layernorm_fwd")


def layernorm_bwd(dy, x, gamma, mean, rstd, rows, D, *, lddy, ldx, lddx, dres=None, dx=None, dx_bf16=None,
                  dgamma=None, dbeta=None):
    for n_, t_ in (("x", x), ("gamma", gamma), ("mean", mean), ("rstd", rstd),
                   ("dx", dx), ("dgamma", dgamma), ("dbeta", dbeta)):
        _chk(t_, F32, n_)
    _chk(dx_bf16, BF16, "dx_bf16")
    _chk(dy, dy.dtype if dy.dtype in (F32, BF16) else F32, "dy")
    if dres is not None:
        _chk(dres, dres.dtype if dres.dtype in (F32, BF16) else F32, "dres")
    check(load_library().aim_layernorm_bwd(dy.data_ptr(), int(dy.dtype == BF16), lddy, x.data_ptr(), ldx, gamma.data_ptr(),
                                           mean.data_ptr(), rstd.data_ptr(), _p(dres),
                                           int(dres is not None and dres.dtype == BF16), _p(dx), _p(dx_bf16), lddx,
                                           _p(dgamma), _p(dbeta), rows, D, _stream()), "aim_layernorm_bwd")


LN_FSUM_GROUPS = 13


def layernorm_bwd_fsum(dy, x, gamma, mean, rstd, dres, dx_bf16, w, partial, frames, ntok, D):
    _chk(dy, BF16, "dy"); _chk(dres, BF16, "dres"); _chk(dx_bf16, BF16, "dx_bf16")
    for n_, t_ in (("x", x), ("gamma", gamma), ("mean", mean), ("rstd", rstd), ("w", w), ("partial", partial)):
        _chk(t_, F32, n_)
    assert partial.numel() >= frames * LN_FSUM_GROUPS * D
    check(load_library().aim_layernorm_bwd_fsum(dy.data_ptr(), D, x.data_ptr(), D, gamma.data_ptr(), mean.data_ptr(),
                                                rstd.data_ptr(), dres.data_ptr(), dx_bf16.data_ptr(), D, _p(w),
                                                partial.data_ptr(), LN_FSUM_GROUPS, frames, ntok, D, _stream()),
          "aim_layernorm_bwd_fsum")


def attn_fwd(qkv, out, lse, BT, N, H):
    _chk(qkv, BF16, "qkv"); _chk(out, BF16, "out"); _chk(lse, F32, "lse")
    check(load_library().aim_attn_fwd(qkv.data_ptr(), out.data_ptr(), lse.data_ptr(), BT, N, H, _stream()),
          "aim_attn_fwd")


def attn_bwd(qkv, out, dout, lse, delta, dqkv, BT, N, H):
    _chk(qkv, BF16, "qkv"); _chk(out, BF16, "out"); _chk(dout, BF16, "dout"); _chk(dqkv, BF16, "dqkv")
    _chk(lse, F32, "lse"); _chk(delta, F32, "delta")
    check(load_library().aim_attn_bwd(qkv.data_ptr(), out.data_ptr(), dout.data_ptr(), lse.data_ptr(),
                                      delta.data_ptr(), dqkv.data_ptr(), BT, N, H, _stream()), "aim_attn_bwd")


def cls_attn_fwd(qkv, out_cls, probs, B, T, N, H):
    _chk(qkv, BF16, "qkv"); _chk(out_cls, BF16, "out_cls"); _chk(probs, F32, "probs")
    check(load_library().aim_cls_attn_fwd(qkv.data_ptr(), out_cls.data_ptr(), probs.data_ptr(), B, T, N, H,
                                          _stream()), "aim_cls_attn_fwd")


def cls_attn_bwd(qkv, probs, dout_cls, dqkv, B, T, N, H, compact: bool = False):
    _chk(qkv, BF16, "qkv"); _chk(dout_cls, BF16, "dout_cls"); _chk(dqkv, BF16, "dqkv"); _chk(probs, F32, "probs")
    check(load_library().aim_cls_attn_bwd(qkv.data_ptr(), probs.data_ptr(), dout_cls.data_ptr(), dqkv.data_ptr(),
                                          int(compact), B, T, N, H, _stream()), "aim_cls_attn_bwd")


def tattn_fwd(qkv, out, probs, B, T, N, H):
    _chk(qkv, BF16, "qkv"); _chk(out, BF16, "out"); _chk(probs, F32, "probs")
    check(load_library().aim_tattn_fwd(qkv.data_ptr(), out.data_ptr(), probs.data_ptr(), B, T, N, H, _stream()), "aim_tattn_fwd")


def tattn_bwd(qkv, probs, dout, dqkv, B, T, N, H):
    _chk(qkv, BF16, "qkv"); _chk(probs, F32, "probs"); _chk(dout, BF16, "dout"); _chk(dqkv, BF16, "dqkv")
    check(load_library().aim_tattn_bwd(qkv.data_ptr(), probs.data_ptr(), dout.data_ptr(), dqkv.data_ptr(), B, T, N, H, _stream()),
          "aim_tattn_bwd")


def add_bf16(a, b, out):
    _chk(a, BF16, "a"); _chk(b, BF16, "b"); _chk(out, BF16, "out")
    R, C = a.shape
    check(load_library().aim_add_bf16(a.data_ptr(), a.stride(0), b.data_ptr(), b.stride(0), out.data_ptr(), out.stride(0), R, C,
                                      _stream()), "aim_add_bf16")
    return out


def acc_bf16(x, s):
    _chk(x, F32, "x"); _chk(s, BF16, "s")
    assert x.is_contiguous() and x.shape == s.shape
    check(load_library().aim_acc_bf16(x.data_ptr(), s.data_ptr(), s.stride(0), x.shape[0], x.shape[1], _stream()), "aim_acc_bf16")
    return x


def lambda_partials(partials, lam, one_minus, BT):
    _chk(partials, F32, "partials"); _chk(lam, F32, "lam"); _chk(one_minus, F32, "one_minus")
    check(load_library().aim_lambda_partials(partials.data_ptr(), lam.data_ptr(), _p(one_minus), BT, _stream()),
          "aim_lambda_partials")


def qk_cross(qkv, kx, ss, BT, N, D, scale):
    _chk(qkv, BF16, "qkv"); _chk(kx, BF16, "kx"); _chk(ss, F32, "ss")
    check(load_library().aim_qk_cross(qkv.data_ptr(), kx.data_ptr(), kx.stride(0), ss.data_ptr(), BT, N, D, scale,
                                      _stream()), "aim_qk_cross")


def qk_border(qkv, kx, ss, partials, slot0: int, BT, N, D, scale):
    _chk(qkv, BF16, "qkv"); _chk(kx, BF16, "kx"); _chk(ss, F32, "ss"); _chk(partials, F32, "partials")
    assert partials.dim() == 3 and partials.shape[0] == BT and partials.shape[2] == 2 and partials.is_contiguous()
    check(load_library().aim_qk_border(qkv.data_ptr(), kx.data_ptr(), kx.stride(0), ss.data_ptr(), partials.data_ptr(), slot0,
                                       partials.shape[1], BT, N, D, scale, _stream()), "aim_qk_border")


def lambda_(qkv, kx, partials, ntiles, lam, one_minus, BT, N, D, scale, ss=None):
    _chk(qkv, BF16, "qkv"); _chk(kx, BF16, "kx"); _chk(partials, F32, "partials"); _chk(lam, F32, "lam")
    _chk(one_minus, F32, "one_minus"); _chk(ss, F32, "ss")
    check(load_library().aim_lambda(qkv.data_ptr(), kx.data_ptr(), kx.stride(0), _p(ss), partials.data_ptr(), ntiles,
                                    lam.data_ptr(), _p(one_minus), BT, N, D, scale, _stream()), "aim_lambda")


_IN_DTYPES = {torch.float32: 0, torch.uint8: 1, torch.bfloat16: 2}


def patchify(imgs, A, B, T, H, W, p, Kp, mean3=None, std3=None):
    if imgs.dtype not in _IN_DTYPES:
        raise TypeError(f"patchify: unsupported input dtype {imgs.dtype} (float32, uint8, bfloat16)")
    if not imgs.is_cuda or not imgs.is_contiguous():
        raise ValueError("patchify: imgs must be a contiguous GPU tensor")
    _chk(A, BF16, "A"); _chk(mean3, F32, "mean3"); _chk(std3, F32, "std3")
    check(load_library().aim_patchify(imgs.data_ptr(), _IN_DTYPES[imgs.dtype], _p(mean3), _p(std3), A.data_ptr(),
                                      B, T, H, W, p, Kp, _stream()), "aim_patchify")


def embed_ln(tok, cls, pos, temporal, gamma, beta, x, mean, rstd, B, T, N, D, eps=1e-5):
    _chk(tok, BF16, "tok")
    for n_, t_ in (("cls", cls), ("pos", pos), ("temporal", temporal), ("gamma", gamma), ("beta", beta), ("x", x),
                   ("mean", mean), ("rstd", rstd)):
        _chk(t_, F32, n_)
    check(load_library().aim_embed_ln(tok.data_ptr(), cls.data_ptr(), pos.data_ptr(), temporal.data_ptr(),
                                      gamma.data_ptr(), beta.data_ptr(), x.data_ptr(), mean.data_ptr(),
                                      rstd.data_ptr(), B, T, N, D, eps, _stream()), "aim_embed_ln")


def embed_bwd(dx, tok, cls, pos, temporal, gamma, mean, rstd, dtemporal, B, T, N, D):
    _chk(tok, BF16, "tok")
    for n_, t_ in (("cls", cls), ("pos", pos), ("temporal", temporal), ("gamma", gamma), ("mean", mean),
                   ("rstd", rstd), ("dtemporal", dtemporal)):
        _chk(t_, F32, n_)
    _chk(dx, dx.dtype if dx.dtype in (F32, BF16) else F32, "dx")
    lib = load_library()
    nbytes = lib.aim_embed_bwd_workspace_bytes(B, T, N, D)
    ws = torch.empty((nbytes // 4,), dtype=F32, device=dx.device)
    check(lib.aim_embed_bwd(dx.data_ptr(), int(dx.dtype == BF16), tok.data_ptr(), cls.data_ptr(), pos.data_ptr(),
                            temporal.data_ptr(), gamma.data_ptr(), mean.data_ptr(), rstd.data_ptr(),
                            dtemporal.data_ptr(), B, T, N, D, ws.data_ptr(), nbytes, _stream()), "aim_embed_bwd")


def embed_nopre_fwd(tok, cls, pos, temporal, x, B, T, N, D):
    for n_, t_ in (("tok", tok), ("cls", cls), ("pos", pos), ("temporal", temporal), ("x", x)):
        _chk(t_, F32, n_)
    check(load_library().aim_embed_nopre_fwd(tok.data_ptr(), cls.data_ptr(), pos.data_ptr(), temporal.data_ptr(), x.data_ptr(),
                                             B, T, N, D, _stream()), "aim_embed_nopre_fwd")


def embed_nopre_bwd(dx, B, T, N, D, *, dtok=None, dcls=None, dpos=None, dtemporal=None, dbias=None):
    _chk(dx, dx.dtype if dx.dtype in (F32, BF16) else F32, "dx")
    _chk(dtok, dx.dtype, "dtok")
    for n_, t_ in (("dcls", dcls), ("dpos", dpos), ("dtemporal", dtemporal), ("dbias", dbias)):
        _chk(t_, F32, n_)
    assert dx.is_contiguous() and (dtok is None or dtok.is_contiguous())
    lib = load_library()
    nbytes = lib.aim_embed_nopre_bwd_workspace_bytes(B, T, N, D)
    ws = torch.empty((nbytes // 4,), dtype=F32, device=dx.device)
    check(lib.aim_embed_nopre_bwd(dx.data_ptr(), int(dx.dtype == BF16), _p(dtok), _p(dcls), _p(dpos), _p(dtemporal), _p(dbias),
                                  B, T, N, D, ws.data_ptr(), nbytes, _stream()), "aim_embed_nopre_bwd")


def layernorm_gb_bwd(dy, x, mean, rstd, rows, D, dgamma, dbeta, *, lddy=None, ldx=None):
    _chk(dy, dy.dtype if dy.dtype in (F32, BF16) else F32, "dy")
    for n_, t_ in (("x", x), ("mean", mean), ("rstd", rstd), ("dgamma", dgamma), ("dbeta", dbeta)):
        _chk(t_, F32, n_)
    lib = load_library()
    nbytes = lib.aim_layernorm_gb_bwd_workspace_bytes(rows, D)
    ws = torch.empty((nbytes // 4,), dtype=F32, device=dy.device)
    check(lib.aim_layernorm_gb_bwd(dy.data_ptr(), int(dy.dtype == BF16), dy.stride(0) if lddy is None else lddy, x.data_ptr(),
                                   x.stride(0) if ldx is None else ldx, mean.data_ptr(), rstd.data_ptr(), _p(dgamma), _p(dbeta),
                                   rows, D, ws.data_ptr(), nbytes, _stream()), "aim_layernorm_gb_bwd")


def frame_sum(x, w, out, frames, ntok, D):
    _chk(x, x.dtype if x.dtype in (F32, BF16) else F32, "x"); _chk(w, F32, "w"); _chk(out, F32, "out")
    check(load_library().aim_frame_sum(x.data_ptr(), int(x.dtype == BF16), _p(w), out.data_ptr(), frames, ntok, D, _stream()),
          "aim_frame_sum")


def colsum(X, out, *, af=None, at=None, ntok=0):
    _chk(X, BF16, "X"); _chk(out, F32, "out"); _chk(af, F32, "af"); _chk(at, F32, "at")
    ws = None
    if X.shape[0] > 64:
        ws = torch.empty((min(1024, (X.shape[0] + 63) // 64), X.shape[1]), dtype=F32, device=X.device)
    check(load_library().aim_colsum_bf16(X.data_ptr(), X.stride(0), _p(af), _p(at), ntok, out.data_ptr(),
                                         X.shape[0], X.shape[1], _p(ws), ws.numel() * 4 if ws is not None else 0,
                                         _stream()), "aim_colsum_bf16")


def cast_bf16(src, dst, transpose=False):
    _chk(src, F32, "src"); _chk(dst, BF16, "dst")
    R, C = src.shape
    assert tuple(dst.shape) == ((C, R) if transpose else (R, C)) and src.is_contiguous()
    check(load_library().aim_cast_bf16(src.data_ptr(), dst.data_ptr(), R, C, int(transpose), dst.stride(0), _stream()),
          "aim_cast_bf16")


def scale_rows(x, s, y=None, y_f32=None):
    _chk(x, F32, "x"); _chk(s, F32, "s"); _chk(y, BF16, "y"); _chk(y_f32, F32, "y_f32")
    R, C = x.shape
    check(load_library().aim_scale_rows(x.data_ptr(), s.data_ptr(), _p(y), _p(y_f32), R, C, _stream()),
          "aim_scale_rows")


def add_rows(dst, dst_row_stride: int, src):
    _chk(dst, BF16, "dst"); _chk(src, F32, "src")
    R, C = src.shape
    check(load_library().aim_add_rows_bf16(dst.data_ptr(), int(dst_row_stride), src.data_ptr(), R, C, _stream()),
          "aim_add_rows_bf16")


def adamw_flat(p, g, m, v, lr, beta1, beta2, eps, weight_decay, step, grad_scale: float = 1.0):
    for n_, t_ in (("p", p), ("g", g), ("m", m), ("v", v)):
        _chk(t_, F32, n_)
    check(load_library().aim_adamw_flat(p.data_ptr(), g.data_ptr(), m.data_ptr(), v.data_ptr(), p.numel(), lr, beta1,
                                        beta2, eps, weight_decay, step, grad_scale, _stream()), "aim_adamw_flat")


def head_fwd(feat, drop, W, bias):
    _chk(feat, F32, "feat"); _chk(drop, F32, "drop"); _chk(W, F32, "W"); _chk(bias, F32, "bias")
    B, T, D = feat.shape
    C = W.shape[0]
    assert feat.is_contiguous() and W.is_contiguous() and W.shape[1] == D
    pooled = torch.empty((B, D), dtype=F32, device=feat.device)
    score = torch.empty((B, C), dtype=F32, device=feat.device)
    check(load_library().aim_head_fwd(feat.data_ptr(), _p(drop), W.data_ptr(), _p(bias), pooled.data_ptr(),
                                      score.data_ptr(), B, T, D, C, _stream()), "aim_head_fwd")
    return pooled, score


def head_bwd(dscore, pooled, drop, W, T, need_dfeat=True):
    _chk(dscore, F32, "dscore"); _chk(pooled, F32, "pooled"); _chk(drop, F32, "drop"); _chk(W, F32, "W")
    B, C = dscore.shape
    D = W.shape[1]
    assert dscore.is_contiguous() and pooled.is_contiguous()
    dW = torch.zeros((C, D), dtype=F32, device=W.device)
    db = torch.zeros((C,), dtype=F32, device=W.device)
    dfeat = torch.empty((B, T, D), dtype=F32, device=W.device) if need_dfeat else None
    check(load_library().aim_head_bwd(dscore.data_ptr(), pooled.data_ptr(), _p(drop), W.data_ptr(), dW.data_ptr(),
                                      db.data_ptr(), _p(dfeat), B, T, D, C, _stream()), "aim_head_bwd")
    return dW, db, dfeat


def ce_soft(score, label, class_weight=None, need_grad: bool = True):
    _chk(score, F32, "score"); _chk(label, F32, "label"); _chk(class_weight, F32, "class_weight")
    B, C = score.shape
    assert score.is_contiguous() and label.is_contiguous() and label.shape == score.shape
    assert class_weight is None or (class_weight.is_contiguous() and class_weight.numel() == C)
    dscore = torch.empty_like(score) if need_grad else None
    ws = torch.empty((B, 2), dtype=F32, device=score.device)
    out = torch.empty((1,), dtype=F32, device=score.device)
    check(load_library().aim_ce_soft(score.data_ptr(), label.data_ptr(), _p(class_weight), _p(dscore), ws.data_ptr(),
                                     out.data_ptr(), B, C, _stream()), "aim_ce_soft")
    return out, dscore


def ce_topk(score, label, k2: int = 5, need_grad: bool = True):
    _chk(score, F32, "score")
    if label.dtype != torch.int64 or not label.is_cuda:
        raise TypeError("ce_topk: label must be an int64 GPU tensor")
    B, C = score.shape
    assert score.is_contiguous() and label.numel() == B
    dscore = torch.empty_like(score) if need_grad else None
    ws = torch.empty((B, 4), dtype=F32, device=score.device)
    out3 = torch.empty((3,), dtype=F32, device=score.device)
    check(load_library().aim_ce_topk(score.data_ptr(), label.data_ptr(), _p(dscore), ws.data_ptr(), out3.data_ptr(), B, C,
                                     k2, _stream()), "aim_ce_topk")
    return out3, dscore


class CastTable:

    def __init__(self, entries, device):
        import struct
        self.keep = entries
        raw = b"".join(struct.pack("<QQiiii", src.data_ptr(), dst.data_ptr(), src.shape[0], src.shape[1], dst.stride(0),
                                   int(tr)) for src, dst, tr in entries)
        for src, dst, tr in entries:
            _chk(src, F32, "src"); _chk(dst, F32 if tr == 2 else BF16, "dst")
            assert src.dim() == 2 and src.is_contiguous() and src.numel() < 2 ** 31
            assert tuple(dst.shape) == ((src.shape[1], src.shape[0]) if tr is True or tr == 1 else tuple(src.shape))
        self.n = len(entries)
        self.table = torch.frombuffer(bytearray(raw), dtype=torch.uint8).to(device)
        self.ptrs = tuple(src.data_ptr() for src, _, _ in entries)

    def run(self):
        check(load_library().aim_cast_multi(self.table.data_ptr(), self.n, _stream()), "aim_cast_multi")


def gemm_f32(a: torch.Tensor, w: torch.Tensor, epi: int, out: torch.Tensor, *, bias=None, resid=None, af=None, at=None,
             vec=None, bt=None, ntok: int = 0, act: int = 0, n_split: int = 0, act2: int = 0, ldv: Optional[int] = None,
             batch: int = 1, stride_a: int = 0, stride_w: int = 0, M: Optional[int] = None, N: Optional[int] = None,
             K: Optional[int] = None, lda: Optional[int] = None, ldw: Optional[int] = None, ldo: Optional[int] = None,
             out2=None, aux=None):
    for n_, t_ in (("a", a), ("w", w), ("out", out), ("bias", bias), ("resid", resid), ("af", af), ("at", at), ("vec", vec), ("bt", bt),
                   ("out2", out2), ("aux", aux)):
        _chk(t_, F32, n_)
    g = GemmArgs()
    g.A, g.W = a.data_ptr(), w.data_ptr()
    g.M = a.shape[0] if M is None else M
    g.K = a.shape[1] if K is None else K
    g.N = w.shape[0] if N is None else N
    g.lda = a.stride(0) if lda is None else lda
    g.ldw = w.stride(0) if ldw is None else ldw
    g.strideA, g.strideW = stride_a, stride_w
    g.bias, g.resid = _p(bias), _p(resid)
    g.ldr = resid.stride(0) if resid is not None else 0
    g.af, g.at, g.vec, g.bt = _p(af), _p(at), _p(vec), _p(bt)
    g.ldv = (vec.stride(0) if ldv is None else ldv) if vec is not None else 0
    g.ntok = ntok
    g.out = out.data_ptr()
    g.ldo = (out.stride(-2) if out.dim() >= 2 else g.N) if ldo is None else ldo
    g.act, g.n_split, g.act2, g.scale = act, n_split, act2, 1.0
    if out2 is not None:
        g.out2, g.ldo2 = out2.data_ptr(), out2.stride(0)
    if aux is not None:
        g.aux, g.ldaux = aux.data_ptr(), aux.stride(0)
    check(load_library().aim_gemm_f32(byref(g), epi, batch, _stream()), "aim_gemm_f32")
    return out


def attn_fwd_f32(qkv, out, BT, N, H):
    _chk(qkv, F32, "qkv"); _chk(out, F32, "out")
    check(load_library().aim_attn_fwd_f32(qkv.data_ptr(), out.data_ptr(), BT, N, H, _stream()), "aim_attn_fwd_f32")


def cls_attn_fwd_f32(qkv, row_stride: int, out_cls, B, T, H):
    _chk(qkv, F32, "qkv"); _chk(out_cls, F32, "out_cls")
    check(load_library().aim_cls_attn_fwd_f32(qkv.data_ptr(), int(row_stride), out_cls.data_ptr(), B, T, H, _stream()),
          "aim_cls_attn_fwd_f32")


def lambda_f32(scores, qkv, kx, lam, one_minus, BT, N, D, scale):
    for n_, t_ in (("scores", scores), ("qkv", qkv), ("kx", kx), ("lam", lam), ("one_minus", one_minus)):
        _chk(t_, F32, n_)
    check(load_library().aim_lambda_f32(scores.data_ptr(), scores.stride(-2), qkv.data_ptr(), kx.data_ptr(), kx.stride(0),
                                        lam.data_ptr(), _p(one_minus), BT, N, D, scale, _stream()), "aim_lambda_f32")


def _blend_args(imgs, B, blend):
    if imgs.dtype not in (torch.float32, torch.uint8):
        raise TypeError(f"patchify_blend: unsupported input dtype {imgs.dtype} (float32, uint8)")
    if not imgs.is_cuda or not imgs.is_contiguous():
        raise ValueError("patchify_blend: imgs must be a contiguous GPU tensor")
    _chk(blend.partner, torch.int32, "partner")
    if blend.partner.numel() != B or not blend.partner.is_contiguous():
        raise ValueError(f"patchify_blend: partner must hold one index per clip ({B}), got {tuple(blend.partner.shape)}")
    x1, y1, x2, y2 = blend.box
    return (blend.partner.data_ptr(), blend.mode, blend.lam, blend.oml, x1, y1, x2, y2)


def patchify_blend(imgs, A, B, T, H, W, p, Kp, mean3=None, std3=None, blend=None):
    args = _blend_args(imgs, B, blend)
    _chk(A, BF16, "A"); _chk(mean3, F32, "mean3"); _chk(std3, F32, "std3")
    check(load_library().aim_patchify_blend(imgs.data_ptr(), _IN_DTYPES[imgs.dtype], _p(mean3), _p(std3), A.data_ptr(),
                                            B, T, H, W, p, Kp, *args, _stream()), "aim_patchify_blend")


def patchify_blend_f32(imgs, A, B, T, H, W, p, Kp, mean3=None, std3=None, blend=None):
    args = _blend_args(imgs, B, blend)
    _chk(A, F32, "A"); _chk(mean3, F32, "mean3"); _chk(std3, F32, "std3")
    check(load_library().aim_patchify_blend_f32(imgs.data_ptr(), _IN_DTYPES[imgs.dtype], _p(mean3), _p(std3), A.data_ptr(),
                                                B, T, H, W, p, Kp, *args, _stream()), "aim_patchify_blend_f32")


def patchify_f32(imgs, A, B, T, H, W, p, Kp, mean3=None, std3=None):
    if imgs.dtype not in (torch.float32, torch.uint8):
        raise TypeError(f"patchify_f32: unsupported input dtype {imgs.dtype} (float32, uint8)")
    if not imgs.is_cuda or not imgs.is_contiguous():
        raise ValueError("patchify_f32: imgs must be a contiguous GPU tensor")
    _chk(A, F32, "A"); _chk(mean3, F32, "mean3"); _chk(std3, F32, "std3")
    check(load_library().aim_patchify_f32(imgs.data_ptr(), _IN_DTYPES[imgs.dtype], _p(mean3), _p(std3), A.data_ptr(), B, T, H, W,
                                          p, Kp, _stream()), "aim_patchify_f32")


def embed_ln_f32(tok, cls, pos, temporal, gamma, beta, x, B, T, N, D, eps=1e-5, pre=None, mean=None, rstd=None):
    for n_, t_ in (("tok", tok), ("cls", cls), ("pos", pos), ("temporal", temporal), ("gamma", gamma), ("beta", beta), ("x", x),
                   ("pre", pre), ("mean", mean), ("rstd", rstd)):
        _chk(t_, F32, n_)
    check(load_library().aim_embed_ln_f32(tok.data_ptr(), cls.data_ptr(), pos.data_ptr(), temporal.data_ptr(), gamma.data_ptr(),
                                          beta.data_ptr(), x.data_ptr(), _p(pre), _p(mean), _p(rstd), B, T, N, D, eps, _stream()),
          "aim_embed_ln_f32")


def attn_bwd_f32(qkv, dout, dqkv, BT, N, H):
    for n_, t_ in (("qkv", qkv), ("dout", dout), ("dqkv", dqkv)):
        _chk(t_, F32, n_)
    lib = load_library()
    nbytes = lib.aim_attn_bwd_f32_workspace_bytes(BT, N, H)
    ws = torch.empty((nbytes // 4,), dtype=F32, device=qkv.device)
    check(lib.aim_attn_bwd_f32(qkv.data_ptr(), dout.data_ptr(), dqkv.data_ptr(), BT, N, H, ws.data_ptr(), nbytes, _stream()),
          "aim_attn_bwd_f32")


def cls_attn_bwd_f32(qkv, row_stride: int, dout_cls, dqkv, B, T, H):
    for n_, t_ in (("qkv", qkv), ("dout_cls", dout_cls), ("dqkv", dqkv)):
        _chk(t_, F32, n_)
    check(load_library().aim_cls_attn_bwd_f32(qkv.data_ptr(), int(row_stride), dout_cls.data_ptr(), dqkv.data_ptr(), B, T, H,
                                              _stream()), "aim_cls_attn_bwd_f32")


def tattn_fwd_f32(qkv, out, B, T, N, H):
    _chk(qkv, F32, "qkv"); _chk(out, F32, "out")
    check(load_library().aim_tattn_fwd_f32(qkv.data_ptr(), out.data_ptr(), B, T, N, H, _stream()), "aim_tattn_fwd_f32")


def tattn_bwd_f32(qkv, dout, dqkv, B, T, N, H):
    for n_, t_ in (("qkv", qkv), ("dout", dout), ("dqkv", dqkv)):
        _chk(t_, F32, n_)
    check(load_library().aim_tattn_bwd_f32(qkv.data_ptr(), dout.data_ptr(), dqkv.data_ptr(), B, T, N, H, _stream()),
          "aim_tattn_bwd_f32")


def wgrad_f32(g, a, dw, db=None, at=None, ntok: int = 0):
    for n_, t_ in (("g", g), ("a", a), ("dw", dw), ("db", db), ("at", at)):
        _chk(t_, F32, n_)
    M, Nw = g.shape
    Kw = a.shape[1]
    assert a.shape[0] == M and tuple(dw.shape) == (Nw, Kw) and dw.is_contiguous() and g.stride(1) == 1 and a.stride(1) == 1
    lib = load_library()
    nbytes = lib.aim_wgrad_f32_workspace_bytes(M, Nw, Kw)
    ws = torch.empty((nbytes // 4,), dtype=F32, device=g.device)
    check(lib.aim_wgrad_f32(g.data_ptr(), g.stride(0), a.data_ptr(), a.stride(0), dw.data_ptr(), M, Nw, Kw, _p(db), _p(at), ntok,
                            ws.data_ptr(), nbytes, _stream()), "aim_wgrad_f32")
```

### include/aim_kernels.h

```cpp
#ifndef AIM_KERNELS_H
#define AIM_KERNELS_H

#include <stdint.h>

#ifdef __cplusplus
extern "C" {
#endif

typedef uint16_t aim_bf16;

#define AIM_ABI_VERSION 8

int aim_version(void);
const char* aim_last_error(void);

enum {
    AIM_EPI_BF16 = 0,
    AIM_EPI_ACT = 1,
    AIM_EPI_DACT = 2,
    AIM_EPI_F32 = 3,
    AIM_EPI_EXPSUM = 4,
    AIM_EPI_ACT8 = 5,
    AIM_EPI_RES16 = 6
};
enum { AIM_ACT_QGELU = 0, AIM_ACT_GELU = 1 };

typedef struct aim_gemm_args {
    const aim_bf16* A;
    const aim_bf16* W;
    int32_t lda, ldw;
    int64_t strideA, strideW;
    int32_t M, N, K;
    const float* bias;
    const float* resid;
    int32_t ldr;
    const float* af;
    const float* at;
    const float* vec;
    const float* bt;
    int32_t ldv, ntok;
    const aim_bf16* aux;
    int32_t ldaux;
    void* out;  int32_t ldo;
    void* out2; int32_t ldo2;
    float scale;
    int32_t act;
    int32_t rs_bias_only;
    int32_t n_split, act2;
    const aim_bf16* xrow;
    int32_t ldx;
    int32_t reserve_cus;
    void* probe;
    int32_t probe_cap;
    const float* wscale;
    int32_t aux_grad;
    int32_t aux_frag;
    int32_t row0;
} aim_gemm_args;

int aim_gemm_bf16(const aim_gemm_args* args, int epilogue, int batch, void* stream);

int aim_gemm_fp8(const aim_gemm_args* args, int epilogue, void* stream);
int aim_gemm_expsum_tiles(int M, int N);

int aim_wgrad_bf16(const aim_bf16* G, int ldg, const aim_bf16* A, int lda, float* dW, int lddw,
                   float* db, int M, int Nw, int Kw,
                   float* workspace ,
                   int64_t workspace_bytes, void* stream);
int64_t aim_wgrad_workspace_bytes(int M, int Nw, int Kw);
int aim_wgrad_bias_bf16(const aim_bf16* G, int ldg, const aim_bf16* A, int lda, float* dW, int lddw, float* db,
                        const float* at, int ntok, int M, int Nw, int Kw, float* workspace, int64_t workspace_bytes, void* stream);

int aim_layernorm_fwd(const float* x, int64_t ldx, const float* gamma, const float* beta,
                      aim_bf16* y_bf16, float* y_f32, int64_t ldy, float* mean, float* rstd,
                      int rows, int D, float eps, void* stream);
int aim_layernorm_fwd_fp8(const float* x, int64_t ldx, const float* gamma, const float* beta, uint8_t* y_fp8,
                          int64_t ldy, int rows, int D, float eps, void* stream);
int aim_layernorm_fwd_x16(const aim_bf16* x, int64_t ldx, const float* gamma, const float* beta, aim_bf16* y_bf16,
                          float* y_f32, uint8_t* y_fp8, int64_t ldy, int rows, int D, float eps, void* stream);
int aim_layernorm_bwd(const void* dy, int dy_is_bf16 , int64_t lddy,
                      const float* x, int64_t ldx, const float* gamma,
                      const float* mean, const float* rstd, const void* dres, int dres_is_bf16, float* dx,
                      aim_bf16* dx_bf16, int64_t lddx, float* dgamma, float* dbeta,
                      int rows, int D, void* stream);
int aim_layernorm_bwd_fsum(const aim_bf16* dy, int64_t lddy, const float* x, int64_t ldx, const float* gamma,
                           const float* mean, const float* rstd, const aim_bf16* dres, aim_bf16* dx_bf16, int64_t lddx,
                           const float* w, float* fsum_partial, int groups, int frames, int ntok, int D, void* stream);

int aim_attn_fwd(const aim_bf16* qkv, aim_bf16* out, float* lse, int BT, int N, int H, void* stream);
int aim_attn_fwd_fp8(const aim_bf16* qkv, uint8_t* out_fp8, float* lse, int BT, int N, int H, void* stream);
int aim_attn_bwd(const aim_bf16* qkv, const aim_bf16* out, const aim_bf16* dout, const float* lse,
                 float* delta , aim_bf16* dqkv, int BT, int N, int H,
                 void* stream);

int aim_cls_attn_fwd(const aim_bf16* qkv, aim_bf16* out_cls, float* probs, int B, int T, int N, int H,
                     void* stream);
int aim_cls_attn_bwd(const aim_bf16* qkv, const float* probs, const aim_bf16* dout_cls, aim_bf16* dqkv, int compact,
                     int B, int T, int N, int H, void* stream);

int aim_tattn_fwd(const aim_bf16* qkv, aim_bf16* out, float* probs, int B, int T, int N, int H, void* stream);
int aim_tattn_bwd(const aim_bf16* qkv, const float* probs, const aim_bf16* dout, aim_bf16* dqkv, int B, int T, int N, int H,
                  void* stream);
int aim_add_bf16(const aim_bf16* a, int64_t lda, const aim_bf16* b, int64_t ldb, aim_bf16* out, int64_t ldo, int R, int C,
                 void* stream);
int aim_acc_bf16(float* x, const aim_bf16* s, int64_t lds, int R, int C, void* stream);

int aim_lambda_partials(const float* partials, float* lam, float* one_minus_lam, int BT, void* stream);
int aim_qk_cross(const aim_bf16* qkv, const aim_bf16* kx, int ldkx, float* ss, int BT, int N, int D, float scale, void* stream);
int aim_lambda(const aim_bf16* qkv, const aim_bf16* kx, int ldkx, const float* ss, const float* partials, int ntiles,
               float* lam, float* one_minus_lam, int BT, int N, int D, float scale, void* stream);
int aim_qk_border(const aim_bf16* qkv, const aim_bf16* kx, int ldkx, float* ss, float* partials , int slot0,
                  int nslots, int BT, int N, int D, float scale, void* stream);

int aim_patchify(const void* imgs, int in_dtype , const float* mean3, const float* std3, aim_bf16* A,
                 int B, int T, int H, int W, int p, int Kp, void* stream);
int aim_patchify_blend(const void* imgs, int in_dtype, const float* mean3, const float* std3, aim_bf16* A, int B, int T, int H,
                       int W, int p, int Kp, const int32_t* partner, int mode, float lam, float oml, int x1, int y1, int x2,
                       int y2, void* stream);
int aim_embed_ln(const aim_bf16* tok, const float* cls, const float* pos, const float* temporal,
                 const float* gamma, const float* beta, float* x, float* mean, float* rstd,
                 int B, int T, int N, int D, float eps, void* stream);
int aim_embed_bwd(const void* dx, int dx_is_bf16, const aim_bf16* tok, const float* cls, const float* pos,
                  const float* temporal, const float* gamma, const float* mean, const float* rstd,
                  float* dtemporal, int B, int T, int N, int D,
                  float* workspace , int64_t workspace_bytes,
                  void* stream);
int64_t aim_embed_bwd_workspace_bytes(int B, int T, int N, int D);

int aim_frame_sum(const void* x, int x_is_bf16, const float* w, float* out, int frames, int ntok, int D, void* stream);
int aim_colsum_bf16(const aim_bf16* X, int ldx, const float* af, const float* at, int ntok,
                    float* out, int M, int C, float* workspace ,
                    int64_t workspace_bytes, void* stream);
int aim_cast_bf16(const float* src, aim_bf16* dst, int R, int C, int transpose, int ldd ,
                  void* stream);
int aim_scale_rows(const float* x, const float* s, aim_bf16* y, float* y_f32, int R, int C, void* stream);
int aim_add_rows_bf16(aim_bf16* dst, int64_t dst_row_stride, const float* src, int R, int C, void* stream);

typedef struct aim_cast_desc {
    const float* src;
    void* dst;
    int32_t R, C, ldd, transpose;
} aim_cast_desc;
int aim_cast_multi(const aim_cast_desc* table_dev, int n, void* stream);

int aim_adamw_flat(float* p, const float* g, float* m, float* v, int64_t n, float lr, float beta1,
                   float beta2, float eps, float weight_decay, int step, float grad_scale, void* stream);

int aim_head_fwd(const float* feat, const float* drop, const float* W, const float* bias, float* pooled, float* score,
                 int B, int T, int D, int C, void* stream);
int aim_head_bwd(const float* dscore, const float* pooled, const float* drop, const float* W, float* dW, float* db,
                 float* dfeat, int B, int T, int D, int C, void* stream);
int aim_ce_topk(const float* score, const int64_t* label, float* dscore, float* per_sample ,
                float* out3, int B, int C, int k2 , void* stream);
int aim_ce_soft(const float* score, const float* label, const float* class_weight, float* dscore,
                float* per_sample , float* out , int B, int C, void* stream);

int aim_gemm_f32(const aim_gemm_args* args, int epilogue, int batch, void* stream);
int aim_attn_fwd_f32(const float* qkv, float* out, int BT, int N, int H, void* stream);
int aim_cls_attn_fwd_f32(const float* qkv, int64_t row_stride, float* out_cls, int B, int T, int H, void* stream);
int aim_lambda_f32(const float* scores, int lds, const float* qkv, const float* kx, int ldkx, float* lam,
                   float* one_minus_lam, int BT, int N, int D, float scale, void* stream);
int aim_patchify_f32(const void* imgs, int in_dtype, const float* mean3, const float* std3, float* A, int B, int T,
                     int H, int W, int p, int Kp, void* stream);
int aim_patchify_blend_f32(const void* imgs, int in_dtype, const float* mean3, const float* std3, float* A, int B, int T,
                           int H, int W, int p, int Kp, const int32_t* partner, int mode, float lam, float oml, int x1, int y1,
                           int x2, int y2, void* stream);
int aim_embed_ln_f32(const float* tok, const float* cls, const float* pos, const float* temporal, const float* gamma,
                     const float* beta, float* x, float* pre, float* mean, float* rstd, int B, int T, int N, int D, float eps,
                     void* stream);
int64_t aim_attn_bwd_f32_workspace_bytes(int BT, int N, int H);
int aim_attn_bwd_f32(const float* qkv, const float* dout, float* dqkv, int BT, int N, int H, float* workspace,
                     int64_t workspace_bytes, void* stream);
int aim_cls_attn_bwd_f32(const float* qkv, int64_t row_stride, const float* dout_cls, float* dqkv, int B, int T, int H,
                         void* stream);
int aim_tattn_fwd_f32(const float* qkv, float* out, int B, int T, int N, int H, void* stream);
int aim_tattn_bwd_f32(const float* qkv, const float* dout, float* dqkv, int B, int T, int N, int H, void* stream);
int64_t aim_wgrad_f32_workspace_bytes(int M, int Nw, int Kw);
int aim_wgrad_f32(const float* G, int ldg, const float* A, int lda, float* dW, int M, int Nw, int Kw, float* db,
                  const float* at, int ntok, float* workspace, int64_t workspace_bytes, void* stream);

int aim_embed_nopre_fwd(const float* tok, const float* cls, const float* pos, const float* temporal, float* x, int B, int T,
                        int N, int D, void* stream);
int64_t aim_embed_nopre_bwd_workspace_bytes(int B, int T, int N, int D);
int aim_embed_nopre_bwd(const void* dx, int dx_is_bf16, void* dtok, float* dcls, float* dpos, float* dtemporal, float* dbias,
                        int B, int T, int N, int D, float* workspace, int64_t workspace_bytes, void* stream);
int64_t aim_layernorm_gb_bwd_workspace_bytes(int rows, int D);
int aim_layernorm_gb_bwd(const void* dy, int dy_is_bf16, int64_t lddy, const float* x, int64_t ldx, const float* mean,
                         const float* rstd, float* dgamma, float* dbeta, int rows, int D, float* workspace,
                         int64_t workspace_bytes, void* stream);

#ifdef __cplusplus
}
#endif
#endif
```

Measured before the change: 1289 clips/s.

## Batch per-block adapter weight-gradient GEMMs into a grouped multi-descriptor launch

Adapter weight-gradient calls within a block (MLP adapter fc1/fc2 plus spatial and temporal adapter fc1/fc2) are now gathered into one batch. That batch is issued through a new wgrad_multi entry point, which packs all small-M jobs into a single grouped kernel and merges the split-K finish reductions into one launch. The wgrad kernel is also templated on tile shape, gains XCD-aware block remapping for large-M jobs, and writes directly instead of using atomics when there is a single chunk. The aim is to cut kernel-launch and Python dispatch overhead for the many tiny adapter wgrads and to fill the GPU better. The cost is an ABI bump, a per-call workspace allocation, and a limit of 8 descriptors per batch.

```diff
diff --git a/adapt-image-models_amd/backbone.py b/adapt-image-models_amd/backbone.py
--- a/adapt-image-models_amd/backbone.py
+++ b/adapt-image-models_amd/backbone.py
@@ -531,20 +531,33 @@
     return x2, xn, mean2, rstd2, hcat_pre, a_s
 
 
-def _mlp_adapter_backward(dyb, x_in, mean2, rstd2, xn, hcat_pre, a_s, dms2, fz: _Frozen, gm, N, fsum=None):
+class _WgradBatch:
+
+    def __init__(self):
+        self.calls: list = []
+
+    def add(self, g, a, dw, db, at=None, ntok: int = 0):
+        self.calls.append((g, a, dw, db, at, ntok))
+
+    def __call__(self):
+        if self.calls:
+            ops.wgrad_multi(self.calls)
+
+
+def _mlp_adapter_backward(dyb, x_in, mean2, rstd2, xn, hcat_pre, a_s, dms2, fz: _Frozen, gm, N, fsum=None, batch=None):
     dev = dyb.device
     M, D = dyb.shape
     r, H4 = fz.r, 4 * D
-    big_later: list = []
+    batch = _WgradBatch() if batch is None else batch
     if _DETACH_BIG:
-        big_later.append(lambda: ops.wgrad(dyb, a_s, gm["D_fc2.weight"], gm["D_fc2.bias"], at=dms2, ntok=N))
+        batch.add(dyb, a_s, gm["D_fc2.weight"], gm["D_fc2.bias"], at=dms2, ntok=N)
     else:
         ops.wgrad(dyb, a_s, gm["D_fc2.weight"], gm["D_fc2.bias"], at=dms2, ntok=N)
     dcat = _empty((M, H4 + r), BF16, dev)
     ops.gemm(dyb, fz.WcatT2, ops.EPI_DACT, dcat, aux=hcat_pre, act=ops.ACT_QGELU, n_split=H4, act2=ops.ACT_GELU,
              at=dms2, ntok=N, aux_grad=_AUX_GRAD, aux_frag=_AUX_FRAG and dyb.shape[0] >= 1024, reserve_cus=_DP_RESERVE)
     if _DETACH_BIG:
-        big_later.append(lambda: ops.wgrad(dcat[:, H4:], xn, gm["D_fc1.weight"], gm["D_fc1.bias"]))
+        batch.add(dcat[:, H4:], xn, gm["D_fc1.weight"], gm["D_fc1.bias"])
     else:
         ops.wgrad(dcat[:, H4:], xn, gm["D_fc1.weight"], gm["D_fc1.bias"])
     dxn = _empty((M, D), BF16, dev)
@@ -554,14 +567,15 @@
         ops.layernorm_bwd_fsum(dxn, x_in, fz.g2, mean2, rstd2, dyb, dxb, fsum[0], fsum[1], M // N, N, D)
     else:
         ops.layernorm_bwd(dxn, x_in, fz.g2, mean2, rstd2, M, D, lddy=D, ldx=D, lddx=D, dres=dyb, dx_bf16=dxb)
-    return dxb, big_later
-
-
-def _adapter_bwd_small(dout_bf, ad: _AdapterW, a_in, pre, h, grads, rows, r, D, ar: _Arena, need_dx_bf16: bool, later: list):
-    later.append(lambda: ops.wgrad(dout_bf, h, grads["D_fc2.weight"], grads["D_fc2.bias"]))
+    return dxb, [batch] if batch.calls else []
+
+
+def _adapter_bwd_small(dout_bf, ad: _AdapterW, a_in, pre, h, grads, rows, r, D, ar: _Arena, need_dx_bf16: bool,
+                       later: _WgradBatch):
+    later.add(dout_bf, h, grads["D_fc2.weight"], grads["D_fc2.bias"])
     dpre = ar.take((rows, r), BF16)
     ops.gemm(dout_bf, ad.W2T, ops.EPI_DACT, dpre, aux=pre, act=ops.ACT_GELU, aux_grad=_AUX_GRAD)
-    later.append(lambda: ops.wgrad(dpre, a_in, grads["D_fc1.weight"], grads["D_fc1.bias"]))
+    later.add(dpre, a_in, grads["D_fc1.weight"], grads["D_fc1.bias"])
     din = ar.take((rows, D), BF16 if need_dx_bf16 else F32)
     ops.gemm(dpre, ad.W1T, ops.EPI_BF16 if need_dx_bf16 else ops.EPI_F32, din)
     return din
@@ -573,9 +587,9 @@
     BT = B * T
     r, H4 = fz.r, 4 * D
     fpart = _empty((BT, ops.LN_FSUM_GROUPS, D), F32, dev) if _FSUM_IN_LN else None
-    dx1b, big_later = _mlp_adapter_backward(dyb, c["x1"], c["mean2"], c["rstd2"], c["xn"], c["hcat_pre"], c["a_s"], c["dms2"],
-                                            fz, grads["MLP_Adapter"], N, fsum=(c["dms1"], fpart) if _FSUM_IN_LN else None)
-    later: list = big_later
+    wgb = _WgradBatch()
+    dx1b, _ = _mlp_adapter_backward(dyb, c["x1"], c["mean2"], c["rstd2"], c["xn"], c["hcat_pre"], c["a_s"], c["dms2"],
+                                    fz, grads["MLP_Adapter"], N, fsum=(c["dms1"], fpart) if _FSUM_IN_LN else None, batch=wgb)
     ar = _Arena(dev, 48 * BT * D + (1 << 16))
     with _Fork(dev, "bwd") as fork:
         dsv = ar.take((BT, D), F32)
@@ -586,7 +600,7 @@
         dsv_b = ar.take((BT, D), BF16)
         ops.cast_bf16(dsv, dsv_b)
         dsin = _adapter_bwd_small(dsv_b, adp["S_Adapter"], c["sin"], c["s_pre"], c["s_h"], grads["S_Adapter"], BT, r,
-                                  D, ar, need_dx_bf16=False, later=later)
+                                  D, ar, need_dx_bf16=False, later=wgb)
         dcrs = ar.take((BT, D), BF16)
         ops.scale_rows(dsin, c["lam"], y=dcrs)
         dvx = ar.take((BT, D), BF16)
@@ -594,7 +608,7 @@
         dxt = ar.take((BT, D), BF16)
         ops.gemm(dvx, fz.WqkvT[:, 2 * D:], ops.EPI_BF16, dxt)
         dta = _adapter_bwd_small(dxt, adp["T_Adapter"], c["ta"], c["t_pre"], c["t_h"], grads["T_Adapter"], BT, r, D,
-                                 ar, need_dx_bf16=True, later=later)
+                                 ar, need_dx_bf16=True, later=wgb)
         dot = ar.take((BT, D), BF16)
         ops.gemm(dta, fz.WoT, ops.EPI_BF16, dot)
         if _LATE_JOIN:
@@ -602,6 +616,7 @@
             ops.cls_attn_bwd(c["qkv"], c["probs"], dot, dqkv_cls, B, T, N, H, compact=True)
             dxl_cls = ar.take((BT, D), F32)
             ops.gemm(dqkv_cls, fz.WqkvT, ops.EPI_F32, dxl_cls)
+    later = [wgb]
     if keep is None:
         keep = []
         fork.run_detached(later, keep)
diff --git a/adapt-image-models_amd/csrc/wgrad.hip b/adapt-image-models_amd/csrc/wgrad.hip
--- a/adapt-image-models_amd/csrc/wgrad.hip
+++ b/adapt-image-models_amd/csrc/wgrad.hip
@@ -10,19 +10,19 @@
 constexpr int OPER_BYTES = 4 * IMG;
 constexpr int STAGE_BYTES = 2 * OPER_BYTES;
 constexpr int TILE = 256;
-
-__global__ __launch_bounds__(512) void wgrad_kernel(const bf16_t* __restrict__ G, int ldg, const bf16_t* __restrict__ A,
-                                                    int lda, float* __restrict__ dW, int lddw, float* __restrict__ partial,
-                                                    int M, int Nw, int Kw, int chunk, float* __restrict__ db,
-                                                    float* __restrict__ bias_partial, const float* __restrict__ at, int ntok) {
-    extern __shared__ __attribute__((aligned(16))) char smem_raw[];
-    AIM_LDS char* smem = (AIM_LDS char*)smem_raw;
+constexpr int SMALL_M = 1024;
+constexpr int MAX_DESC = 8;
+
+template <int TN, int TK>
+__device__ __forceinline__ void wgrad_tile(AIM_LDS char* smem, int cidx, int tn, int tk, const bf16_t* __restrict__ G,
+                                           int ldg, const bf16_t* __restrict__ A, int lda, float* __restrict__ dW, int lddw,
+                                           float* __restrict__ partial, int M, int Nw, int Kw, int chunk,
+                                           float* __restrict__ db, float* __restrict__ bias_partial,
+                                           const float* __restrict__ at, int ntok) {
+    constexpr int WN = TN / 2, WK = TK / 4;
+    constexpr int FN = WN / 16, FK = WK / 16;
     AIM_LDS float* sAt = (AIM_LDS float*)(smem + NST * STAGE_BYTES);
-    const int tiles_k = (Kw + TILE - 1) / TILE;
-    const int tiles = ((Nw + TILE - 1) / TILE) * tiles_k;
-    const int cidx = blockIdx.x / tiles, tix = blockIdx.x - cidx * tiles;
-    const int tn = tix / tiles_k, tk = tix - tn * tiles_k;
-    const int n0 = tn * TILE, k0 = tk * TILE;
+    const int n0 = tn * TN, k0 = tk * TK;
     const int mbeg = cidx * chunk;
     const int mend = min(M, mbeg + chunk);
     if (mbeg >= mend) return;
@@ -35,8 +35,8 @@
     const bf16_t* Gb = G + (long long)mbeg * ldg + n0;
     const bf16_t* Ab = A + (long long)mbeg * lda + k0;
     const int rows = mend - mbeg;
-    aim_rsrc_words rG = make_rsrc_words(Gb, ((long long)(rows - 1) * ldg + min(TILE, Nw - n0)) * 2);
-    aim_rsrc_words rA = make_rsrc_words(Ab, ((long long)(rows - 1) * lda + min(TILE, Kw - k0)) * 2);
+    aim_rsrc_words rG = make_rsrc_words(Gb, ((long long)(rows - 1) * ldg + min(TN, Nw - n0)) * 2);
+    aim_rsrc_words rA = make_rsrc_words(Ab, ((long long)(rows - 1) * lda + min(TK, Kw - k0)) * 2);
 
     const int srow = lane >> 3, schunk = (lane & 7) ^ srow;
     unsigned vg0[2], va0[2];
@@ -47,8 +47,8 @@
         const int img = piece >> 2, rg = piece & 3;
         const int r = rg * 8 + srow;
         const int col = img * 64 + schunk * 8;
-        vg0[j] = n0 + col < Nw ? (unsigned)((r * ldg + col) * 2) : AIM_OOB;
-        va0[j] = k0 + col < Kw ? (unsigned)((r * lda + col) * 2) : AIM_OOB;
+        vg0[j] = (col < TN && n0 + col < Nw) ? (unsigned)((r * ldg + col) * 2) : AIM_OOB;
+        va0[j] = (col < TK && k0 + col < Kw) ? (unsigned)((r * lda + col) * 2) : AIM_OOB;
         pdst[j] = smem + img * IMG + rg * 1024;
     }
     const unsigned gstep = (unsigned)(MSTEP * ldg * 2), astep = (unsigned)(MSTEP * lda * 2);
@@ -60,11 +60,11 @@
         }
     };
 
-    f32x4 acc[8][4];
-#pragma unroll
-    for (int i = 0; i < 8; ++i)
-#pragma unroll
-        for (int j = 0; j < 4; ++j) acc[i][j] = f32x4{0.f, 0.f, 0.f, 0.f};
+    f32x4 acc[FN][FK];
+#pragma unroll
+    for (int i = 0; i < FN; ++i)
+#pragma unroll
+        for (int j = 0; j < FK; ++j) acc[i][j] = f32x4{0.f, 0.f, 0.f, 0.f};
 
     auto frag = [&](const AIM_LDS char* oper, int c0) -> bf16x8 {
         const AIM_LDS char* img = oper + (c0 >> 6) * IMG;
@@ -114,25 +114,26 @@
 #pragma unroll
             for (int e = 0; e < 8; ++e) bs[e] += f0 * (float)v0[e] + f1 * (float)v1[e];
         }
-        bf16x8 gf[8], af[4];
-#pragma unroll
-        for (int j = 0; j < 4; ++j) af[j] = frag(sA, wk * 64 + j * 16);
-#pragma unroll
-        for (int i = 0; i < 8; ++i) gf[i] = frag(sG, wn * 128 + i * 16);
-#pragma unroll
-        for (int i = 0; i < 8; ++i)
-#pragma unroll
-            for (int j = 0; j < 4; ++j)
+        bf16x8 gf[FN], af[FK];
+#pragma unroll
+        for (int j = 0; j < FK; ++j) af[j] = frag(sA, wk * WK + j * 16);
+#pragma unroll
+        for (int i = 0; i < FN; ++i) gf[i] = frag(sG, wn * WN + i * 16);
+#pragma unroll
+        for (int i = 0; i < FN; ++i)
+#pragma unroll
+            for (int j = 0; j < FK; ++j)
                 acc[i][j] = __builtin_amdgcn_mfma_f32_16x16x32_bf16(af[j], gf[i], acc[i][j], 0, 0, 0);
     }
     asm volatile("s_waitcnt vmcnt(0)" ::: "memory");
+    const bool direct = chunk >= M;
     if (do_bias) {
         __syncthreads();
         AIM_LDS float* red = (AIM_LDS float*)smem;
 #pragma unroll
         for (int e = 0; e < 8; ++e) red[brow * 256 + bcg * 8 + e] = bs[e];
         __syncthreads();
-        if (tid < 256 && n0 + tid < Nw) {
+        if (tid < TN && n0 + tid < Nw) {
             float v = 0.f;
 #pragma unroll
             for (int r = 0; r < 16; ++r) v += red[r * 256 + tid];
@@ -142,125 +143,324 @@
     }
     float* slab = partial ? partial + (long long)cidx * Nw * Kw : nullptr;
 #pragma unroll
-    for (int i = 0; i < 8; ++i)
-#pragma unroll
-        for (int j = 0; j < 4; ++j) {
-            const int n = n0 + wn * 128 + i * 16 + frow;
-            const int k = k0 + wk * 64 + j * 16 + fq * 4;
+    for (int i = 0; i < FN; ++i)
+#pragma unroll
+        for (int j = 0; j < FK; ++j) {
+            const int n = n0 + wn * WN + i * 16 + frow;
+            const int k = k0 + wk * WK + j * 16 + fq * 4;
             if (n >= Nw || k >= Kw) continue;
             if (slab) *(f32x4*)(slab + (long long)n * Kw + k) = acc[i][j];
-            else
+            else if (direct) {
+                f32x4* o = (f32x4*)(dW + (long long)n * lddw + k);
+                *o = *o + acc[i][j];
+            } else
 #pragma unroll
                 for (int e = 0; e < 4; ++e) atomicAdd(dW + (long long)n * lddw + k + e, acc[i][j][e]);
         }
 }
 
-__global__ __launch_bounds__(256) void wgrad_finish_kernel(const float* __restrict__ partial, float* __restrict__ dW,
-                                                           int lddw, int nchunks, int Nw, int Kw,
-                                                           const float* __restrict__ bias_partial, float* __restrict__ db) {
-    const long long total = (long long)Nw * Kw;
-    const long long idx = ((long long)blockIdx.x * 256 + threadIdx.x) * 4;
+template <int TN, int TK>
+__global__ __launch_bounds__(512) void wgrad_kernel(const bf16_t* __restrict__ G, int ldg, const bf16_t* __restrict__ A,
+                                                    int lda, float* __restrict__ dW, int lddw, float* __restrict__ partial,
+                                                    int M, int Nw, int Kw, int chunk, float* __restrict__ db,
+                                                    float* __restrict__ bias_partial, const float* __restrict__ at, int ntok,
+                                                    int xcd) {
+    extern __shared__ __attribute__((aligned(16))) char smem_raw[];
+    const int tiles_k = (Kw + TK - 1) / TK;
+    const int tiles = ((Nw + TN - 1) / TN) * tiles_k;
+    const int b = blockIdx.x;
+    int cidx, tix;
+    if (xcd) {
+        const int s = b >> 3, l = s / tiles;
+        tix = s - l * tiles;
+        cidx = l * 8 + (b & 7);
+    } else {
+        cidx = b / tiles;
+        tix = b - cidx * tiles;
+    }
+    const int tn = tix / tiles_k, tk = tix - tn * tiles_k;
+    wgrad_tile<TN, TK>((AIM_LDS char*)smem_raw, cidx, tn, tk, G, ldg, A, lda, dW, lddw, partial, M, Nw, Kw, chunk, db,
+                       bias_partial, at, ntok);
+}
+
+struct SmallJob {
+    const bf16_t* G;
+    const bf16_t* A;
+    float* dW;
+    float* db;
+    const float* at;
+    float* partial;
+    float* bias_partial;
+    int ldg, lda, lddw, ntok, M, Nw, Kw, tiles, tiles_k, chunk, wg0;
+};
+struct SmallBatch {
+    SmallJob j[MAX_DESC];
+    int n;
+};
+
+__global__ __launch_bounds__(512) void wgrad_small_kernel(const SmallBatch batch) {
+    extern __shared__ __attribute__((aligned(16))) char smem_raw[];
+    const int b = blockIdx.x;
+    SmallJob J = batch.j[0];
+#pragma unroll
+    for (int i = 1; i < MAX_DESC; ++i)
+        if (i < batch.n && b >= batch.j[i].wg0) J = batch.j[i];
+    const int local = b - J.wg0;
+    const int cidx = local / J.tiles, tix = local - cidx * J.tiles;
+    const int tn = tix / J.tiles_k, tk = tix - tn * J.tiles_k;
+    wgrad_tile<TILE, TILE>((AIM_LDS char*)smem_raw, cidx, tn, tk, J.G, J.ldg, J.A, J.lda, J.dW, J.lddw, J.partial, J.M, J.Nw,
+                           J.Kw, J.chunk, J.db, J.bias_partial, J.at, J.ntok);
+}
+
+struct FinishJob {
+    const float* partial;
+    const float* bias_partial;
+    float* dW;
+    float* db;
+    int lddw, nchunks, Nw, Kw, wg0;
+};
+struct FinishBatch {
+    FinishJob j[MAX_DESC];
+    int n;
+};
+
+__global__ __launch_bounds__(256) void wgrad_finish_kernel(const FinishBatch batch) {
+    FinishJob J = batch.j[0];
+#pragma unroll
+    for (int i = 1; i < MAX_DESC; ++i)
+        if (i < batch.n && (int)blockIdx.x >= batch.j[i].wg0) J = batch.j[i];
+    const int blk = (int)blockIdx.x - J.wg0;
+    const long long total = (long long)J.Nw * J.Kw;
+    const long long idx = ((long long)blk * 256 + threadIdx.x) * 4;
     if (idx < total) {
         f32x4 acc = f32x4{0.f, 0.f, 0.f, 0.f};
         int c = 0;
-        for (; c + 8 <= nchunks; c += 8) {
+        for (; c + 8 <= J.nchunks; c += 8) {
             f32x4 v[8];
 #pragma unroll
-            for (int j = 0; j < 8; ++j) v[j] = *(const f32x4*)(partial + (long long)(c + j) * total + idx);
+            for (int j = 0; j < 8; ++j) v[j] = *(const f32x4*)(J.partial + (long long)(c + j) * total + idx);
 #pragma unroll
             for (int j = 0; j < 8; ++j) acc += v[j];
         }
-        for (; c < nchunks; ++c) acc += *(const f32x4*)(partial + (long long)c * total + idx);
-        const int n = (int)(idx / Kw), k = (int)(idx - (long long)n * Kw);
-        f32x4* o = (f32x4*)(dW + (long long)n * lddw + k);
+        for (; c < J.nchunks; ++c) acc += *(const f32x4*)(J.partial + (long long)c * total + idx);
+        const int n = (int)(idx / J.Kw), k = (int)(idx - (long long)n * J.Kw);
+        f32x4* o = (f32x4*)(J.dW + (long long)n * J.lddw + k);
         *o = *o + acc;
     }
-    if (bias_partial) {
-        const int n = blockIdx.x * 4 + (threadIdx.x >> 6), lane = threadIdx.x & 63;
-        if (n < Nw) {
+    if (J.bias_partial) {
+        const int n = blk * 4 + (threadIdx.x >> 6), lane = threadIdx.x & 63;
+        if (n < J.Nw) {
             float a = 0.f;
-            for (int c = lane; c < nchunks; c += 64) a += bias_partial[(long long)c * Nw + n];
+            for (int c = lane; c < J.nchunks; c += 64) a += J.bias_partial[(long long)c * J.Nw + n];
             a = wave_sum(a);
-            if (lane == 0) db[n] += a;
-        }
-    }
-}
-
-__global__ __launch_bounds__(256) void wgrad_finish1_kernel(const float* __restrict__ partial, float* __restrict__ dW,
-                                                            int lddw, int nchunks, int Nw, int Kw) {
-    const long long idx = (long long)blockIdx.x * 256 + threadIdx.x;
-    const long long total = (long long)Nw * Kw;
-    if (idx >= total) return;
-    float acc = 0.f;
-    for (int c = 0; c < nchunks; ++c) acc += partial[(long long)c * total + idx];
-    const int n = (int)(idx / Kw), k = (int)(idx - (long long)n * Kw);
-    dW[(long long)n * lddw + k] += acc;
-}
-
-}
-
-static int wgrad_chunks(int M, int tiles, int* chunk_out) {
+            if (lane == 0) J.db[n] += a;
+        }
+    }
+}
+
+}
+
+namespace {
+
+struct WgradPlan {
+    int tn, tk, tiles, nchunks, chunk, grid, xcd;
+    int64_t slab_bytes;
+};
+
+WgradPlan wgrad_plan(int M, int Nw, int Kw) {
     static const int target = [] { const char* e = getenv("AIM_WGRAD_WGS"); const int v = e ? atoi(e) : 256; return v > 0 ? v : 256; }();
-    int nchunks = (target + tiles - 1) / tiles;
+    static const bool xcd_on = [] { const char* e = getenv("AIM_WGRAD_XCD"); return !e || atoi(e) != 0; }();
+    WgradPlan p{};
+    p.tn = Nw == 192 ? 192 : TILE;
+    p.tk = (Kw == 192 && p.tn == TILE) ? 192 : TILE;
+    p.tiles = ((Nw + p.tn - 1) / p.tn) * ((Kw + p.tk - 1) / p.tk);
     const int maxchunks = (M + MSTEP - 1) / MSTEP;
-    if (nchunks > maxchunks) nchunks = maxchunks;
-    int chunk = (M + nchunks - 1) / nchunks;
-    chunk = ((chunk + MSTEP - 1) / MSTEP) * MSTEP;
-    if (chunk_out) *chunk_out = chunk;
-    return (M + chunk - 1) / chunk;
+    if (M <= SMALL_M) {
+        static const int split = [] { const char* e = getenv("AIM_WGRAD_SMALL_SPLIT"); const int v = e ? atoi(e) : 4; return v > 0 ? v : 4; }();
+        p.tn = p.tk = TILE;
+        p.tiles = ((Nw + TILE - 1) / TILE) * ((Kw + TILE - 1) / TILE);
+        p.nchunks = split;
+    } else if (p.tn != p.tk && xcd_on) {
+        const int per_xcd = target / (8 * p.tiles);
+        p.nchunks = 8 * (per_xcd > 0 ? per_xcd : 1);
+        p.xcd = 1;
+    } else {
+        p.nchunks = (target + p.tiles - 1) / p.tiles;
+    }
+    if (p.nchunks > maxchunks) p.nchunks = maxchunks;
+    p.chunk = (M + p.nchunks - 1) / p.nchunks;
+    p.chunk = ((p.chunk + MSTEP - 1) / MSTEP) * MSTEP;
+    p.nchunks = (M + p.chunk - 1) / p.chunk;
+    p.grid = p.xcd ? 8 * ((p.nchunks + 7) / 8) * p.tiles : p.nchunks * p.tiles;
+    p.slab_bytes = p.nchunks > 1 ? (int64_t)p.nchunks * Nw * (Kw + 1) * 4 : 0;
+    return p;
+}
+
+int64_t align256(int64_t b) { return (b + 255) & ~(int64_t)255; }
+
+int check_desc(const aim_wgrad_desc& d) {
+    AIM_CHECK_ARG(d.M > 0 && d.Nw > 0 && d.Kw > 0 && (d.Nw % 8) == 0 && (d.Kw % 8) == 0, "wgrad: Nw/Kw must be positive multiples of 8 (Nw=%d Kw=%d)", d.Nw, d.Kw);
+    AIM_CHECK_ARG((d.ldg % 8) == 0 && (d.lda % 8) == 0 && (d.lddw % 4) == 0, "wgrad: ldg/lda must be multiples of 8, lddw of 4");
+    AIM_CHECK_ARG(d.G && d.A && d.dW, "wgrad: null pointer");
+    AIM_CHECK_ARG(!d.at || (d.db && d.ntok > 0 && d.ntok <= 4096), "wgrad: row factors need db and 0 < ntok <= 4096");
+    const int rows = wgrad_plan(d.M, d.Nw, d.Kw).chunk;
+    AIM_CHECK_ARG((long long)rows * (d.ldg > d.lda ? d.ldg : d.lda) * 2 < 0x7fffffffLL, "wgrad: chunk too large");
+    return 0;
+}
+
+int lds_bytes_for(const float* at, int ntok) { return NST * STAGE_BYTES + (at ? ((ntok * 4 + 15) & ~15) : 0); }
+
+template <int TN, int TK>
+void set_lds_attr() {
+    static bool done = false;
+    if (!done) {
+        (void)hipFuncSetAttribute((const void*)wgrad_kernel<TN, TK>, hipFuncAttributeMaxDynamicSharedMemorySize, 160 * 1024);
+        done = true;
+    }
+}
+
+int launch_large(const aim_wgrad_desc& d, const WgradPlan& p, float* slab, float* bias_slab, float* db, hipStream_t stream) {
+    const int lds = lds_bytes_for(d.at, d.ntok);
+    const bf16_t* G = (const bf16_t*)d.G;
+    const bf16_t* A = (const bf16_t*)d.A;
+#define AIM_WGRAD_LAUNCH(TN, TK)                                                                                            \
+    set_lds_attr<TN, TK>();                                                                                                 \
+    hipLaunchKernelGGL((wgrad_kernel<TN, TK>), dim3(p.grid), dim3(512), lds, stream, G, d.ldg, A, d.lda, d.dW, d.lddw, slab, \
+                       d.M, d.Nw, d.Kw, p.chunk, db, bias_slab, d.at, d.ntok, p.xcd)
+    if (p.tn == 192) { AIM_WGRAD_LAUNCH(192, 256); }
+    else if (p.tk == 192) { AIM_WGRAD_LAUNCH(256, 192); }
+    else { AIM_WGRAD_LAUNCH(256, 256); }
+#undef AIM_WGRAD_LAUNCH
+    AIM_CHECK_LAUNCH("aim_wgrad_bf16");
+    return 0;
+}
+
+int launch_small(const aim_wgrad_desc* const* ds, float* const* slabs, float* const* bias_slabs, float* const* dbs, int n,
+                 hipStream_t stream) {
+    static bool attr_set = false;
+    if (!attr_set) {
+        (void)hipFuncSetAttribute((const void*)wgrad_small_kernel, hipFuncAttributeMaxDynamicSharedMemorySize, 160 * 1024);
+        attr_set = true;
+    }
+    SmallBatch b{};
+    int wgs = 0, lds = NST * STAGE_BYTES;
+    for (int i = 0; i < n; ++i) {
+        const aim_wgrad_desc& d = *ds[i];
+        const WgradPlan p = wgrad_plan(d.M, d.Nw, d.Kw);
+        const int tiles_k = (d.Kw + TILE - 1) / TILE;
+        b.j[i] = SmallJob{(const bf16_t*)d.G, (const bf16_t*)d.A, d.dW, dbs[i], d.at, slabs[i], bias_slabs[i], d.ldg, d.lda,
+                          d.lddw, d.ntok, d.M, d.Nw, d.Kw, p.tiles, tiles_k, p.chunk, wgs};
+        wgs += p.tiles * p.nchunks;
+        const int l = lds_bytes_for(d.at, d.ntok);
+        if (l > lds) lds = l;
+    }
+    b.n = n;
+    hipLaunchKernelGGL(wgrad_small_kernel, dim3(wgs), dim3(512), lds, stream, b);
+    AIM_CHECK_LAUNCH("aim_wgrad_bf16(small)");
+    return 0;
+}
+
+int launch_finish(const FinishJob* jobs, int n, hipStream_t stream) {
+    FinishBatch b{};
+    int wgs = 0;
+    for (int i = 0; i < n; ++i) {
+        b.j[i] = jobs[i];
+        b.j[i].wg0 = wgs;
+        const long long total = (long long)jobs[i].Nw * jobs[i].Kw;
+        int g = (int)((total / 4 + 255) / 256);
+        if (jobs[i].bias_partial && (jobs[i].Nw + 3) / 4 > g) g = (jobs[i].Nw + 3) / 4;
+        wgs += g;
+    }
+    b.n = n;
+    hipLaunchKernelGGL(wgrad_finish_kernel, dim3(wgs), dim3(256), 0, stream, b);
+    AIM_CHECK_LAUNCH("aim_wgrad_bf16(finish)");
+    return 0;
+}
+
 }
 
 extern "C" int64_t aim_wgrad_workspace_bytes(int M, int Nw, int Kw) {
-    const int tiles = ((Nw + TILE - 1) / TILE) * ((Kw + TILE - 1) / TILE);
-    const int nchunks = wgrad_chunks(M, tiles, nullptr);
-    return nchunks > 1 ? (int64_t)nchunks * Nw * (Kw + 1) * 4 : 0;
+    if (M <= 0 || Nw <= 0 || Kw <= 0) return 0;
+    return wgrad_plan(M, Nw, Kw).slab_bytes;
 }
 
 extern "C" int aim_wgrad_bias_bf16(const aim_bf16* G, int ldg, const aim_bf16* A, int lda, float* dW, int lddw, float* db,
                                    const float* at, int ntok, int M, int Nw, int Kw, float* workspace, int64_t workspace_bytes,
                                    void* stream) {
-    AIM_CHECK_ARG(M > 0 && Nw > 0 && Kw > 0 && (Nw % 8) == 0 && (Kw % 8) == 0, "wgrad: Nw/Kw must be positive multiples of 8 (Nw=%d Kw=%d)", Nw, Kw);
-    AIM_CHECK_ARG((ldg % 8) == 0 && (lda % 8) == 0 && (lddw % 4) == 0, "wgrad: ldg/lda must be multiples of 8, lddw of 4");
-    AIM_CHECK_ARG(G && A && dW, "wgrad: null pointer");
-    AIM_CHECK_ARG(!at || (db && ntok > 0 && ntok <= 4096), "wgrad: row factors need db and 0 < ntok <= 4096");
-    const int tiles = ((Nw + TILE - 1) / TILE) * ((Kw + TILE - 1) / TILE);
-    int chunk = 0;
-    const int nchunks = wgrad_chunks(M, tiles, &chunk);
-    const int lds_bytes = NST * STAGE_BYTES + (at ? ((ntok * 4 + 15) & ~15) : 0);
-    static bool attr_set = false;
-    if (!attr_set) {
-        (void)hipFuncSetAttribute((const void*)wgrad_kernel, hipFuncAttributeMaxDynamicSharedMemorySize, 160 * 1024);
-        attr_set = true;
-    }
-    AIM_CHECK_ARG((long long)chunk * (ldg > lda ? ldg : lda) * 2 < 0x7fffffffLL, "wgrad: chunk too large");
-    float* slab = (workspace && nchunks > 1 && workspace_bytes >= (int64_t)nchunks * Nw * (Kw + 1) * 4) ? workspace : nullptr;
+    const aim_wgrad_desc d{G, A, dW, db, at, ldg, lda, lddw, ntok, M, Nw, Kw, 0};
+    if (int rc = check_desc(d)) return rc;
+    const hipStream_t s = (hipStream_t)stream;
+    const WgradPlan p = wgrad_plan(M, Nw, Kw);
+    float* slab = (workspace && p.nchunks > 1 && workspace_bytes >= p.slab_bytes) ? workspace : nullptr;
     static const bool fuse_bias = [] { const char* e = getenv("AIM_WGRAD_FUSE_BIAS"); return !e || atoi(e) != 0; }();
-    static const bool finish_v = [] { const char* e = getenv("AIM_WGRAD_FINISH_V"); return !e || atoi(e) != 0; }();
-    float* bias_slab = (slab && db && fuse_bias) ? slab + (long long)nchunks * Nw * Kw : nullptr;
-    if (db && nchunks > 1 && !bias_slab) {
+    float* bias_slab = (slab && db && fuse_bias) ? slab + (long long)p.nchunks * Nw * Kw : nullptr;
+    if (db && p.nchunks > 1 && !bias_slab) {
         const int rc = aim_colsum_bf16(G, ldg, nullptr, at, ntok, db, M, Nw, nullptr, 0, stream);
         if (rc) return rc;
         db = nullptr;
     }
-    hipLaunchKernelGGL(wgrad_kernel, dim3(tiles * nchunks), dim3(512), lds_bytes, (hipStream_t)stream,
-                       (const bf16_t*)G, ldg, (const bf16_t*)A, lda, dW, lddw, slab, M, Nw, Kw, chunk, db, bias_slab, at, ntok);
-    AIM_CHECK_LAUNCH("aim_wgrad_bf16");
-    if (slab) {
-        const long long total = (long long)Nw * Kw;
-        unsigned fgrid = (unsigned)((total / 4 + 255) / 256);
-        if (bias_slab && (unsigned)((Nw + 3) / 4) > fgrid) fgrid = (unsigned)((Nw + 3) / 4);
-        if (finish_v || bias_slab)
-            hipLaunchKernelGGL(wgrad_finish_kernel, dim3(fgrid), dim3(256), 0, (hipStream_t)stream,
-                               slab, dW, lddw, nchunks, Nw, Kw, bias_slab, db);
-        else
-            hipLaunchKernelGGL(wgrad_finish1_kernel, dim3((unsigned)((total + 255) / 256)), dim3(256), 0, (hipStream_t)stream,
-                               slab, dW, lddw, nchunks, Nw, Kw);
-        AIM_CHECK_LAUNCH("aim_wgrad_bf16(finish)");
-    }
-    return 0;
+    if (M <= SMALL_M) {
+        const aim_wgrad_desc* one = &d;
+        if (int rc = launch_small(&one, &slab, &bias_slab, &db, 1, s)) return rc;
+    } else if (int rc = launch_large(d, p, slab, bias_slab, db, s)) {
+        return rc;
+    }
+    if (!slab) return 0;
+    const FinishJob job{slab, bias_slab, dW, db, lddw, p.nchunks, Nw, Kw, 0};
+    return launch_finish(&job, 1, s);
 }
 
 extern "C" int aim_wgrad_bf16(const aim_bf16* G, int ldg, const aim_bf16* A, int lda, float* dW, int lddw, float* db,
                               int M, int Nw, int Kw, float* workspace, int64_t workspace_bytes, void* stream) {
     return aim_wgrad_bias_bf16(G, ldg, A, lda, dW, lddw, db, nullptr, 0, M, Nw, Kw, workspace, workspace_bytes, stream);
 }
+
+extern "C" int64_t aim_wgrad_multi_workspace_bytes(const aim_wgrad_desc* descs, int n) {
+    int64_t bytes = 0;
+    for (int i = 0; descs && i < n; ++i)
+        if (descs[i].M > 0 && descs[i].Nw > 0 && descs[i].Kw > 0)
+            bytes += align256(wgrad_plan(descs[i].M, descs[i].Nw, descs[i].Kw).slab_bytes);
+    return bytes;
+}
+
+extern "C" int aim_wgrad_multi_bf16(const aim_wgrad_desc* descs, int n, float* workspace, int64_t workspace_bytes,
+                                    void* stream) {
+    AIM_CHECK_ARG(descs && n > 0 && n <= MAX_DESC, "wgrad_multi: 1..%d calls per batch (n=%d)", MAX_DESC, n);
+    for (int i = 0; i < n; ++i)
+        if (int rc = check_desc(descs[i])) return rc;
+    const int64_t need = aim_wgrad_multi_workspace_bytes(descs, n);
+    AIM_CHECK_ARG(need == 0 || (workspace && workspace_bytes >= need), "wgrad_multi: workspace smaller than aim_wgrad_multi_workspace_bytes()");
+    const hipStream_t s = (hipStream_t)stream;
+    float* slab[MAX_DESC];
+    float* bias_slab[MAX_DESC];
+    float* dbs[MAX_DESC];
+    FinishJob jobs[MAX_DESC];
+    int njobs = 0;
+    int64_t off = 0;
+    for (int i = 0; i < n; ++i) {
+        const aim_wgrad_desc& d = descs[i];
+        const WgradPlan p = wgrad_plan(d.M, d.Nw, d.Kw);
+        slab[i] = p.nchunks > 1 ? (float*)((char*)workspace + off) : nullptr;
+        bias_slab[i] = (slab[i] && d.db) ? slab[i] + (long long)p.nchunks * d.Nw * d.Kw : nullptr;
+        dbs[i] = d.db;
+        off += align256(p.slab_bytes);
+        if (slab[i]) jobs[njobs++] = FinishJob{slab[i], bias_slab[i], d.dW, d.db, d.lddw, p.nchunks, d.Nw, d.Kw, 0};
+    }
+    const aim_wgrad_desc* small[MAX_DESC];
+    float *sslab[MAX_DESC], *sbias[MAX_DESC], *sdb[MAX_DESC];
+    int nsmall = 0;
+    for (int i = 0; i < n; ++i)
+        if (descs[i].M <= SMALL_M) {
+            small[nsmall] = &descs[i];
+            sslab[nsmall] = slab[i];
+            sbias[nsmall] = bias_slab[i];
+            sdb[nsmall++] = dbs[i];
+        }
+    if (nsmall)
+        if (int rc = launch_small(small, sslab, sbias, sdb, nsmall, s)) return rc;
+    for (int i = 0; i < n; ++i)
+        if (descs[i].M > SMALL_M)
+            if (int rc = launch_large(descs[i], wgrad_plan(descs[i].M, descs[i].Nw, descs[i].Kw), slab[i], bias_slab[i], dbs[i], s))
+                return rc;
+    return njobs ? launch_finish(jobs, njobs, s) : 0;
+}
diff --git a/adapt-image-models_amd/lib.py b/adapt-image-models_amd/lib.py
--- a/adapt-image-models_amd/lib.py
+++ b/adapt-image-models_amd/lib.py
@@ -31,6 +31,14 @@
     ]
 
 
+class WgradDesc(Structure):
+    _fields_ = [
+        ("G", c_void_p), ("A", c_void_p), ("dW", c_void_p), ("db", c_void_p), ("at", c_void_p),
+        ("ldg", c_int32), ("lda", c_int32), ("lddw", c_int32), ("ntok", c_int32),
+        ("M", c_int32), ("Nw", c_int32), ("Kw", c_int32), ("reserved", c_int32),
+    ]
+
+
 P = c_void_p
 I = c_int
 L = c_int64
@@ -45,6 +53,8 @@
     "aim_wgrad_bf16": [P, I, P, I, P, I, P, I, I, I, P, L, P],
     "aim_wgrad_workspace_bytes": [I, I, I],
     "aim_wgrad_bias_bf16": [P, I, P, I, P, I, P, P, I, I, I, I, P, L, P],
+    "aim_wgrad_multi_workspace_bytes": [P, I],
+    "aim_wgrad_multi_bf16": [P, I, P, L, P],
     "aim_layernorm_fwd": [P, L, P, P, P, P, L, P, P, I, I, F, P],
     "aim_layernorm_fwd_fp8": [P, L, P, P, P, L, I, I, F, P],
     "aim_layernorm_fwd_x16": [P, L, P, P, P, P, P, L, I, I, F, P],
@@ -100,7 +110,7 @@
     "aim_layernorm_gb_bwd": [P, I, L, P, L, P, P, P, P, I, I, P, L, P],
 }
 
-ABI_VERSION = 8
+ABI_VERSION = 9
 
 
 def load_library():
diff --git a/adapt-image-models_amd/ops.py b/adapt-image-models_amd/ops.py
--- a/adapt-image-models_amd/ops.py
+++ b/adapt-image-models_amd/ops.py
@@ -3,7 +3,7 @@
 
 import torch
 
-from .lib import GemmArgs, check, load_library
+from .lib import GemmArgs, WgradDesc, check, load_library
 
 EPI_BF16, EPI_ACT, EPI_DACT, EPI_F32, EPI_EXPSUM, EPI_ACT8, EPI_RES16 = 0, 1, 2, 3, 4, 5, 6
 FP8 = torch.float8_e4m3fn
@@ -221,6 +221,20 @@
                                   _p(at), ntok, g.shape[0], g.shape[1], a.shape[1], _p(ws), nbytes, _stream()), "aim_wgrad_bias_bf16")
 
 
+def wgrad_multi(calls):
+    lib = load_library()
+    descs = (WgradDesc * len(calls))()
+    for d, (g, a, dw, db, at, ntok) in zip(descs, calls):
+        _chk(g, BF16, "g"); _chk(a, BF16, "a"); _chk(dw, F32, "dw"); _chk(db, F32, "db"); _chk(at, F32, "at")
+        assert g.shape[0] == a.shape[0] and dw.shape == (g.shape[1], a.shape[1])
+        d.G, d.A, d.dW, d.db, d.at = g.data_ptr(), a.data_ptr(), dw.data_ptr(), _p(db), _p(at)
+        d.ldg, d.lda, d.lddw, d.ntok = g.stride(0), a.stride(0), dw.stride(0), ntok
+        d.M, d.Nw, d.Kw = g.shape[0], g.shape[1], a.shape[1]
+    nbytes = lib.aim_wgrad_multi_workspace_bytes(descs, len(calls))
+    ws = torch.empty(nbytes // 4, dtype=F32, device=calls[0][0].device) if nbytes else None
+    check(lib.aim_wgrad_multi_bf16(descs, len(calls), _p(ws), nbytes, _stream()), "aim_wgrad_multi_bf16")
+
+
 def layernorm_fwd(x, gamma, beta, rows, D, ldx, *, y_bf16=None, y_f32=None, ldy=None, mean=None, rstd=None,
                   eps: float = 1e-5):
     _chk(x, F32, "x"); _chk(gamma, F32, "gamma"); _chk(beta, F32, "beta")
diff --git a/include/aim_kernels.h b/include/aim_kernels.h
--- a/include/aim_kernels.h
+++ b/include/aim_kernels.h
@@ -9,7 +9,7 @@
 
 typedef uint16_t aim_bf16;
 
-#define AIM_ABI_VERSION 8
+#define AIM_ABI_VERSION 9
 
 int aim_version(void);
 const char* aim_last_error(void);
@@ -70,6 +70,16 @@
 int64_t aim_wgrad_workspace_bytes(int M, int Nw, int Kw);
 int aim_wgrad_bias_bf16(const aim_bf16* G, int ldg, const aim_bf16* A, int lda, float* dW, int lddw, float* db,
                         const float* at, int ntok, int M, int Nw, int Kw, float* workspace, int64_t workspace_bytes, void* stream);
+typedef struct aim_wgrad_desc {
+    const aim_bf16* G;
+    const aim_bf16* A;
+    float* dW;
+    float* db;
+    const float* at;
+    int32_t ldg, lda, lddw, ntok, M, Nw, Kw, reserved;
+} aim_wgrad_desc;
+int64_t aim_wgrad_multi_workspace_bytes(const aim_wgrad_desc* descs, int n);
+int aim_wgrad_multi_bf16(const aim_wgrad_desc* descs, int n, float* workspace, int64_t workspace_bytes, void* stream);
 
 int aim_layernorm_fwd(const float* x, int64_t ldx, const float* gamma, const float* beta,
                       aim_bf16* y_bf16, float* y_f32, int64_t ldy, float* mean, float* rstd,
```

New measurement: 1300 clips/s, median of 6. Within noise of the previous version (+0.8%).
